# chrhansk/sleqp

Hardware: AMD Instinct MI355X
Metric: KKT factor+solve/sec (numeric refactor + 1 solve with device-controlled refinement, inputs resident in HBM) (higher is better)
Workload: dtype f64; 1 GPU; banded_n1e5_m5e4; n=100000, m=50000, N=150000, nnz_J=1000000, nnz_tril_K=1100000, nnz_L=11646539, nnz_L_stored=12226637, supernodes=569, etree_levels=10, refine_steps=1, hip_graphs=5, solves_per_factor=1, parallelism=single

## Files before the change

include/hipfact.h:

```cpp
#ifndef HIPFACT_H
#define HIPFACT_H

#include <stddef.h>
#include <stdint.h>

#ifdef __cplusplus
extern "C" {
#endif

#define HIPFACT_VERSION "0.1.0"

enum
{
  HIPFACT_OK         = 0,
  HIPFACT_EINVAL     = -1,
  HIPFACT_EDEVICE    = -2,
  HIPFACT_ESINGULAR  = -3,
  HIPFACT_ENOMEM     = -4,
  HIPFACT_ESTATE     = -5,
  HIPFACT_EINTERNAL  = -6
};

typedef struct hipfact_handle hipfact_handle;

// ... 31 lines not shown
int hipfact_solve_device_multi(hipfact_handle* h, int nrhs, const double* d_rhs, long long ld_rhs,
                               double* d_sol, long long ld_sol, double* omega);

int hipfact_solve_multi(hipfact_handle* h, int nrhs, const double* rhs, double* sol);

enum { HIPFACT_EXTRA_CONVERGED = 0, HIPFACT_EXTRA_STALLED = 1, HIPFACT_EXTRA_NONFINITE = 2, HIPFACT_EXTRA_PASS_LIMIT = 3 };
typedef struct hipfact_extra_info {
  int passes;
  int status;
  double ferr;
  double dz_rel;
  double rho;
  double omega;
} hipfact_extra_info;
int hipfact_solve_device_extra(hipfact_handle* h, const double* d_rhs, double* d_sol, hipfact_extra_info* info );
int hipfact_solve_extra(hipfact_handle* h, const double* rhs, double* sol, hipfact_extra_info* info );

int hipfact_residual_device(hipfact_handle* h, const double* d_b, const double* d_z, double* d_res, int extended);

int hipfact_solve_device_multi_extra(hipfact_handle* h, int nrhs, const double* d_rhs, long long ld_rhs, double* d_sol,
                                     long long ld_sol, hipfact_extra_info* info );
int hipfact_solve_multi_extra(hipfact_handle* h, int nrhs, const double* rhs, double* sol,
                              hipfact_extra_info* info );

int hipfact_residual_device_multi(hipfact_handle* h, int nrhs, const double* d_b, long long ld_b, const double* d_z,
                                  long long ld_z, double* d_res, long long ld_res, int extended);

enum { HIPFACT_COND_STOP_EXACT = 0,
       HIPFACT_COND_STOP_NO_GAIN = 1,
       HIPFACT_COND_STOP_PARALLEL = 2,
       HIPFACT_COND_STOP_MAX_AT_BEST = 3,
       HIPFACT_COND_STOP_REVISIT = 4,
       HIPFACT_COND_STOP_ITMAX = 5 };
typedef struct hipfact_cond_info {
  double norm1;
  double inv_norm1;
  double cond1;
  double omega;
  int exact;
  int iterations;
  int blocks;
  int column;
  int stop;
} hipfact_cond_info;
int hipfact_condition_estimate(hipfact_handle* h, int equilibrated, hipfact_cond_info* info ,
                               double* d_witness );

int hipfact_check(hipfact_handle* h);

int hipfact_synchronize(hipfact_handle* h);

int hipfact_stream(hipfact_handle* h, void** stream);


int hipfact_assemble_kkt(hipfact_handle* h, int n, int m_total, const int* j_colptr, const int* j_rowidx,
                         const double* j_vals, const int* var_index, const int* cons_index, int working_set_size,
                         int* k_nnz, int* k_colptr, int* k_rowidx, double* k_vals);


int hipfact_reduced_matrix(hipfact_handle* h, int* nnz, int* colptr, int* rowidx, double* vals);


typedef struct hipfact_spmat hipfact_spmat;

int hipfact_spmat_create(hipfact_handle* h, int num_rows, int num_cols, const int* colptr, const int* rowidx,
                         const double* vals, hipfact_spmat** out);
int hipfact_spmat_update_values(hipfact_spmat* M, const double* vals);
int hipfact_spmat_free(hipfact_spmat** M);

int hipfact_spmat_mult_vec(hipfact_spmat* M, const double* x, double* y);
int hipfact_spmat_mult_vec_trans(hipfact_spmat* M, const double* x, double* y);
int hipfact_spmat_mult_vec_sym(hipfact_spmat* M, const double* x, double* y);
int hipfact_spmat_mult_device(hipfact_spmat* M, int trans, const double* d_x, double* d_y);


int hipfact_steihaug_solve(hipfact_handle* h, hipfact_spmat* hess, const double* gradient, double trust_radius,
                           double rel_tol, int max_iter, double* newton_step, double* tr_dual, int* iterations);


typedef int (*hipfact_hess_prod_fn)(void* user, const double* direction, double* product);

enum
{
  HIPFACT_TR_STEIHAUG = 0,
  HIPFACT_TR_GLTR     = 1
};

int hipfact_tr_solve(hipfact_handle* h, int method, hipfact_spmat* hess, hipfact_hess_prod_fn prod, void* user,
                     const double* gradient, double trust_radius, double rel_tol, int max_iter, double* newton_step,
                     double* tr_dual, int* iterations);

typedef struct hipfact_tr_extra
{
  double time_limit;
  int timed_out;
  double min_rayleigh;
  double max_rayleigh;
} hipfact_tr_extra;

int hipfact_tr_solve_ex(hipfact_handle* h, int method, hipfact_spmat* hess, hipfact_hess_prod_fn prod, void* user,
                        const double* gradient, double trust_radius, double rel_tol, int max_iter, double* newton_step,
                        double* tr_dual, int* iterations, hipfact_tr_extra* extra);


typedef int (*hipfact_lsqr_prod_fn)(void* user, int trans, const double* in, double* out);

typedef struct hipfact_lsqr_op
{
  int num_residuals;
  hipfact_spmat* jac;
  hipfact_lsqr_prod_fn prod;
  void* user;
  hipfact_spmat* cons;
} hipfact_lsqr_op;

enum
{
  HIPFACT_LSQR_CONVERGED = 0,
  HIPFACT_LSQR_BOUNDARY  = 1,
  HIPFACT_LSQR_MAX_ITER  = 2,
  HIPFACT_LSQR_TIME      = 3,
  HIPFACT_LSQR_ZERO      = 4
};

typedef struct hipfact_lsqr_info
{
  double time_limit;
  int iterations;
  int status;
  int timed_out;
  double phi_bar;
} hipfact_lsqr_info;

int hipfact_lsqr_solve(hipfact_handle* h, const hipfact_lsqr_op* op, const double* rhs, double rel_tol,
                       double trust_radius, double eps, int max_iter, double* step, hipfact_lsqr_info* info);

int hipfact_tridiag_tr(int k, const double* delta, const double* gamma, double gamma0, double radius, double* h,
                       double* lambda);


int hipfact_set_option(hipfact_handle* h, const char* name, double value);

int hipfact_get_info(const hipfact_handle* h, const char* name, double* value);

int hipfact_debug_copy(hipfact_handle* h, const char* name, void* out, size_t bytes);

int hipfact_debug_pool_selftest(int callers, int rounds);

int hipfact_debug_place_rows(int m, const int* Ar_ptr, long long fill_bytes, int classes, long long* bounds, int* classes_out,
                             int* grid_out, int* blocks);
int hipfact_debug_place_items(int nfronts, const int* counts, int classes, int* order, int* lost);

int hipfact_debug_multi_slices(int u, int slice_rows, int* tile_bounds , int cap);

int hipfact_debug_extra_rule(int nblocks, int npasses, const double* dn, const double* zn, int pass_cap, int* applied,
                             int* status, double* ferr, double* rho);
int hipfact_debug_multi_extra_schedule(int ncols, int nblocks, int npasses, const double* dn, const double* zn,
                                       int pass_cap, unsigned int* open_mask, hipfact_extra_info* info);
int hipfact_debug_condest_dense(int N, const double* A, long long ld, hipfact_cond_info* info,
                                double* witness , int* history , int cap);
int hipfact_debug_condest_recorded(int N, int nrecords, const double* records, hipfact_cond_info* info);
enum {
  HIPFACT_CADENCE_FACTOR = 0,
  HIPFACT_CADENCE_SOLVE = 1,
  HIPFACT_CADENCE_VERDICT = 2,
  HIPFACT_CADENCE_JUDGE = 3,
  HIPFACT_CADENCE_RESET = 4,
  HIPFACT_CADENCE_SET_STEPS = 5,
  HIPFACT_CADENCE_SET_CHECK_EVERY = 6,
  HIPFACT_CADENCE_SET_CHECK_BACKOFF = 7,
  HIPFACT_CADENCE_SAVE = 8,
  HIPFACT_CADENCE_RESTORE = 9,
  HIPFACT_CADENCE_DEVICE_RESIDUAL = 10,
  HIPFACT_CADENCE_EVENT_WIDTH = 8,
  HIPFACT_CADENCE_ROW_WIDTH = 20
};
int hipfact_debug_refine_cadence(const int* knobs , int nevents, const double* events, long long* rows);
double hipfact_debug_dd_residual(int nterms, const double* k, const double* z, double b, int lanes);


typedef struct hipfact_plan hipfact_plan;
int hipfact_plan_create(int N, const int* colptr, const int* rowidx, const double* vals ,
                        hipfact_plan** out);
void hipfact_plan_free(hipfact_plan** plan);
const char* hipfact_plan_error(const hipfact_plan* plan);
int hipfact_plan_array(const hipfact_plan* plan, const char* name, const void** data, int64_t* len,
                       int* elem_size);
int hipfact_plan_scalar(const hipfact_plan* plan, const char* name, double* value);

#ifdef __cplusplus
}
#endif

#endif
```

sleqp_amd/_lib.py:

```python
from __future__ import annotations

import ctypes as C
import os

_HERE = os.path.dirname(os.path.abspath(__file__))
LIB_PATH = os.environ.get("HIPFACT_LIBRARY") or os.path.join(_HERE, "csrc", "libhipfact.so")

HIPFACT_OK = 0
ERRORS = {
    -1: "HIPFACT_EINVAL",
    -2: "HIPFACT_EDEVICE",
    -3: "HIPFACT_ESINGULAR",
    -4: "HIPFACT_ENOMEM",
    -5: "HIPFACT_ESTATE",
    -6: "HIPFACT_EINTERNAL",
}

SYMBOLS = [
    "hipfact_create", "hipfact_free", "hipfact_retain", "hipfact_last_error", "hipfact_last_warning", "hipfact_set_matrix", "hipfact_solve_sparse",
    "hipfact_solve_dense", "hipfact_solution", "hipfact_solution_view", "hipfact_condition", "hipfact_refactor_device",
    "hipfact_solve_device", "hipfact_solve_device_multi", "hipfact_solve_multi",
    "hipfact_condition_estimate", "hipfact_debug_condest_dense", "hipfact_debug_condest_recorded",
    "hipfact_solve_device_extra", "hipfact_solve_extra", "hipfact_residual_device", "hipfact_debug_extra_rule", "hipfact_debug_dd_residual",
    "hipfact_solve_device_multi_extra", "hipfact_solve_multi_extra", "hipfact_residual_device_multi", "hipfact_debug_multi_extra_schedule",
    "hipfact_solution_device", "hipfact_synchronize", "hipfact_check", "hipfact_stream",
    "hipfact_assemble_kkt", "hipfact_reduced_matrix", "hipfact_spmat_create", "hipfact_spmat_update_values", "hipfact_spmat_free",
    "hipfact_spmat_mult_vec", "hipfact_spmat_mult_vec_trans", "hipfact_spmat_mult_vec_sym",
    "hipfact_spmat_mult_device", "hipfact_steihaug_solve", "hipfact_tr_solve", "hipfact_tr_solve_ex", "hipfact_lsqr_solve", "hipfact_tridiag_tr", "hipfact_set_option", "hipfact_get_info", "hipfact_debug_copy", "hipfact_debug_pool_selftest",
    "hipfact_debug_place_rows", "hipfact_debug_place_items", "hipfact_debug_multi_slices", "hipfact_debug_refine_cadence", "hipfact_plan_create",
    "hipfact_plan_free", "hipfact_plan_error", "hipfact_plan_array", "hipfact_plan_scalar",
]

_lib = None


class HipfactError(RuntimeError):
    def __init__(self, code: int, message: str):
        super().__init__(f"{ERRORS.get(code, code)}: {message}")
        self.code = code


def load() -> C.CDLL:
    global _lib
    if _lib is not None:
        return _lib
    if not os.path.exists(LIB_PATH):
        raise ImportError(
            f"{LIB_PATH} not found: build the HIP extension first "
            "(python -c 'import __graft_entry__ as g; g.build()' or make -C sleqp_amd/csrc)")
    lib = C.CDLL(LIB_PATH)
    vp, ci, cd = C.c_void_p, C.c_int, C.c_double
    lib.hipfact_create.argtypes = [C.POINTER(vp), ci]
    lib.hipfact_free.argtypes = [C.POINTER(vp)]
    lib.hipfact_retain.argtypes = [vp]
    lib.hipfact_last_error.argtypes = [vp]
    lib.hipfact_last_error.restype = C.c_char_p
    lib.hipfact_last_warning.argtypes = [vp]
    lib.hipfact_last_warning.restype = C.c_char_p
    lib.hipfact_set_matrix.argtypes = [vp, ci, vp, vp, vp]
    lib.hipfact_solve_sparse.argtypes = [vp, ci, ci, vp, vp]
    lib.hipfact_solve_dense.argtypes = [vp, vp]
    lib.hipfact_solution.argtypes = [vp, vp, ci, ci]
    lib.hipfact_solution_view.argtypes = [vp, C.POINTER(vp), ci, ci]
    lib.hipfact_condition.argtypes = [vp, C.POINTER(cd)]
    lib.hipfact_refactor_device.argtypes = [vp, vp]
    lib.hipfact_solve_device.argtypes = [vp, vp, vp]
    lib.hipfact_solve_device_multi.argtypes = [vp, ci, vp, C.c_longlong, vp, C.c_longlong, vp]
    lib.hipfact_solve_multi.argtypes = [vp, ci, vp, vp]
    if hasattr(lib, "hipfact_solve_device_extra"):
        lib.hipfact_solve_device_extra.argtypes = [vp, vp, vp, vp]
        lib.hipfact_solve_extra.argtypes = [vp, vp, vp, vp]
        lib.hipfact_residual_device.argtypes = [vp, vp, vp, vp, ci]
        lib.hipfact_debug_extra_rule.argtypes = [ci, ci, vp, vp, ci, C.POINTER(ci), C.POINTER(ci), C.POINTER(cd), C.POINTER(cd)]
        lib.hipfact_debug_dd_residual.argtypes = [ci, vp, vp, cd, ci]
        lib.hipfact_debug_dd_residual.restype = cd
    if hasattr(lib, "hipfact_solve_device_multi_extra"):
        ll = C.c_longlong
        lib.hipfact_solve_device_multi_extra.argtypes = [vp, ci, vp, ll, vp, ll, vp]
        lib.hipfact_solve_multi_extra.argtypes = [vp, ci, vp, vp, vp]
        lib.hipfact_residual_device_multi.argtypes = [vp, ci, vp, ll, vp, ll, vp, ll, ci]
        lib.hipfact_debug_multi_extra_schedule.argtypes = [ci, ci, ci, vp, vp, ci, vp, vp]
    if hasattr(lib, "hipfact_condition_estimate"):
        lib.hipfact_condition_estimate.argtypes = [vp, ci, vp, vp]
        lib.hipfact_debug_condest_dense.argtypes = [ci, vp, C.c_longlong, vp, vp, vp, ci]
        lib.hipfact_debug_condest_recorded.argtypes = [ci, ci, vp, vp]
    lib.hipfact_solution_device.argtypes = [vp, C.POINTER(vp)]
    lib.hipfact_synchronize.argtypes = [vp]
    lib.hipfact_check.argtypes = [vp]
    lib.hipfact_stream.argtypes = [vp, C.POINTER(vp)]
    lib.hipfact_assemble_kkt.argtypes = [vp, ci, ci, vp, vp, vp, vp, vp, ci, C.POINTER(ci), vp, vp, vp]
    lib.hipfact_reduced_matrix.argtypes = [vp, C.POINTER(ci), vp, vp, vp]
    lib.hipfact_spmat_create.argtypes = [vp, ci, ci, vp, vp, vp, C.POINTER(vp)]
    lib.hipfact_spmat_update_values.argtypes = [vp, vp]
    lib.hipfact_spmat_free.argtypes = [C.POINTER(vp)]
    lib.hipfact_spmat_mult_vec.argtypes = [vp, vp, vp]
    lib.hipfact_spmat_mult_vec_trans.argtypes = [vp, vp, vp]
    lib.hipfact_spmat_mult_vec_sym.argtypes = [vp, vp, vp]
    lib.hipfact_spmat_mult_device.argtypes = [vp, ci, vp, vp]
    lib.hipfact_steihaug_solve.argtypes = [vp, vp, vp, cd, cd, ci, vp, C.POINTER(cd), C.POINTER(ci)]
    lib.hipfact_tr_solve.argtypes = [vp, ci, vp, vp, vp, vp, cd, cd, ci, vp, C.POINTER(cd), C.POINTER(ci)]
    lib.hipfact_tr_solve_ex.argtypes = [vp, ci, vp, vp, vp, vp, cd, cd, ci, vp, C.POINTER(cd), C.POINTER(ci), vp]
    lib.hipfact_lsqr_solve.argtypes = [vp, vp, vp, cd, cd, cd, ci, vp, vp]
    lib.hipfact_tridiag_tr.argtypes = [ci, vp, vp, cd, cd, vp, C.POINTER(cd)]
    lib.hipfact_set_option.argtypes = [vp, C.c_char_p, cd]
    lib.hipfact_debug_copy.argtypes = [vp, C.c_char_p, vp, C.c_size_t]
    lib.hipfact_debug_pool_selftest.argtypes = [ci, ci]
    lib.hipfact_get_info.argtypes = [vp, C.c_char_p, C.POINTER(cd)]
    if hasattr(lib, "hipfact_debug_place_items"):
        lib.hipfact_debug_place_rows.argtypes = [ci, vp, C.c_longlong, ci, vp, C.POINTER(ci), C.POINTER(ci), vp]
        lib.hipfact_debug_place_items.argtypes = [ci, vp, ci, vp, vp]
    if hasattr(lib, "hipfact_debug_multi_slices"):
        lib.hipfact_debug_multi_slices.argtypes = [ci, ci, vp, ci]
    if hasattr(lib, "hipfact_debug_refine_cadence"):
        lib.hipfact_debug_refine_cadence.argtypes = [vp, ci, vp, vp]
    lib.hipfact_plan_create.argtypes = [ci, vp, vp, vp, C.POINTER(vp)]
    lib.hipfact_plan_free.argtypes = [C.POINTER(vp)]
    lib.hipfact_plan_error.argtypes = [vp]
    lib.hipfact_plan_error.restype = C.c_char_p
    lib.hipfact_plan_array.argtypes = [vp, C.c_char_p, C.POINTER(vp), C.POINTER(C.c_int64), C.POINTER(ci)]
    lib.hipfact_plan_scalar.argtypes = [vp, C.c_char_p, C.POINTER(cd)]
    for name in SYMBOLS:
        if not hasattr(lib, name) and not os.environ.get("HIPFACT_LIBRARY"):
            raise ImportError(f"{LIB_PATH} lacks {name}: rebuild it (make -C sleqp_amd/csrc)")
    lib.hipfact_plan_free.restype = None
    _lib = lib
    return lib


def kernel_sources_sha16() -> str:
    import glob
    import hashlib

    d = os.path.join(os.path.dirname(os.path.abspath(__file__)), "csrc")
    h = hashlib.sha256()
    for name in sorted(glob.glob(os.path.join(d, "*.hip")) + glob.glob(os.path.join(d, "*.inc")) + glob.glob(os.path.join(d, "*.h"))):
        h.update(os.path.basename(name).encode())
        h.update(open(name, "rb").read())
    return h.hexdigest()[:16]
```

sleqp_amd/csrc/abi_options.inc:

```
enum OptionEffect {
  FX_NONE,
  FX_GRAPHS,
  FX_GRAPHS_IF_CHANGED,
  FX_PLANS,
  FX_PLANS_IF_CHANGED,
};
struct OptionRow {
  const char* name;
  const char* env;
  OptionEffect effect;
  int (*set)(hipfact_handle* h, double v);
  const char* doc;
};
#define OPT_STORE(field, conv)                 \
  [](hipfact_handle* h, double v) -> int {     \
    const auto x = (conv);                     \
    const bool changed = h->field != x;        \
    h->field = x;                              \
    return changed;                            \
  }
static const OptionRow kOptions[] = {
    {"refine_steps", "HIPFACT_REFINE", FX_GRAPHS,
     [](hipfact_handle* h, double v) -> int {
       h->refine_steps = std::max(0, (int)v);
// ... 138 lines not shown
     "0: hipfact_assemble_kkt analyses every working set on its own rows (no superset plan)"},
    {"plan_cache", nullptr, FX_NONE,
     [](hipfact_handle* h, double v) -> int {
       h->plan_cache_max = std::max(0, (int)v);
       while ((int)h->cache.size() > h->plan_cache_max) h->cache.pop_back();
       return 1;
     },
     "inactive plan states kept (LRU); 0: one pattern at a time"},
    {"profile", nullptr, FX_NONE,
     [](hipfact_handle* h, double v) -> int {
       if (h->prof.on) prof_collect(h);
       if (v < 0)
         for (int c = 0; c < PC_COUNT; ++c) h->prof.ms[c] = 0, h->prof.max_ms[c] = 0, h->prof.cnt[c] = 0;
       h->prof.tagged.clear();
       h->prof.on = v > 0;
       return 1;
     },
     "event-time every kernel class; value < 0 resets the counters"},
    {"ordering", nullptr, FX_PLANS, OPT_STORE(prm.ordering, (int)v),
     "0 nested dissection + AMD leaves (default), 1 AMD on the whole graph, 2 natural"},
    {"max_children", nullptr, FX_PLANS, OPT_STORE(prm.max_children, (int)v),
     "relaxed amalgamation keeps fronts at this many children (default 4 = what the pull extend-add takes in one block)"},
    {"force_generic", nullptr, FX_PLANS, OPT_STORE(prm.force_generic, v != 0.0),
     "1: no saddle-point structure detection, static 1 x 1 pivots on K as given (symmetric positive definite input: the PSD shim)"},
    {"dense_mode", nullptr, FX_PLANS, OPT_STORE(prm.dense_mode, std::min(2, std::max(0, (int)v))),
     "1: late elimination inside the tree (default), 2: low-rank correction, 0: off"},
    {nullptr, "HIPFACT_DATAFLOW_RETRY", FX_NONE, OPT_STORE(df_retry_every, std::max(0, (int)v)), nullptr},
    {nullptr, "HIPFACT_CHECK_LAUNCHES", FX_NONE, OPT_STORE(check_launches, v != 0.0), nullptr},
    {nullptr, "HIPFACT_SOL_SPLIT", FX_NONE, OPT_STORE(sol_split, v != 0.0), nullptr},
    {nullptr, "HIPFACT_XCD_CLASSES", FX_NONE, OPT_STORE(xcd_classes, std::max(1, std::min(XCD_CLASSES_MAX, (int)v))), nullptr},
};
#undef OPT_STORE

static void options_from_environment(hipfact_handle* h) {
  for (const OptionRow& row : kOptions)
    if (const char* s = row.env ? getenv(row.env) : nullptr) (void)row.set(h, (double)atoi(s));
}

int hipfact_set_option(hipfact_handle* h, const char* name, double value) {
  if (!h || !name) return HIPFACT_EINVAL;
  {
    bool known = false;
    const int rc = multi_set_option(h, name, value, known);
    if (known) return rc;
  }
  {
    bool known = false;
    const int rc = condest_set_option(h, name, value, known);
    if (known) return rc;
  }
  for (const OptionRow& row : kOptions) {
    if (!row.name || strcmp(name, row.name)) continue;
    const int changed = row.set(h, value);
    if (changed < 0) return changed;
    if (row.effect == FX_GRAPHS || (row.effect == FX_GRAPHS_IF_CHANGED && changed)) drop_graphs(h);
    if (row.effect == FX_PLANS || (row.effect == FX_PLANS_IF_CHANGED && changed)) invalidate_plans(h);
    return HIPFACT_OK;
  }
  h->error = std::string("unknown option: ") + name;
  return HIPFACT_EINVAL;
}

int hipfact_debug_copy(hipfact_handle* h, const char* name, void* out, size_t bytes) {
  int rc = enter(h);
  if (rc) return rc;
  if (!name || !out) return HIPFACT_EINVAL;
  auto host_copy = [&](const auto& v) {
    if (bytes > v.size() * sizeof(v[0])) {
      h->error = "hipfact_debug_copy: unknown buffer or size";
      return HIPFACT_EINVAL;
    }
    if (bytes) memcpy(out, v.data(), bytes);
    return HIPFACT_OK;
  };
  const Plan& P = h->plan;
  if (!strcmp(name, "perm")) return host_copy(P.perm);
  if (!strcmp(name, "sn_c0")) return host_copy(P.sn_c0);
  if (!strcmp(name, "sn_r")) return host_copy(P.sn_r);
  if (!strcmp(name, "sn_rowptr")) return host_copy(P.sn_rowptr);
  if (!strcmp(name, "sn_rows")) return host_copy(P.sn_rows);
  if (!strcmp(name, "sn_Loff")) return host_copy(P.sn_Loff);
  if (!strcmp(name, "late_cols")) return host_copy(P.late_cols);
  if (!strcmp(name, "sn_level")) return host_copy(P.sn_level);
  if (!strcmp(name, "dense_cols")) return host_copy(P.dense_cols);
  if (!strcmp(name, "cond_history")) return host_copy(h->cond_history);
  const DevBuf* b = nullptr;
  if (!strcmp(name, "L")) b = &h->d_L;
  else if (!strcmp(name, "U")) b = &h->d_U;
  else if (!strcmp(name, "SPf")) b = &h->d_SPf;
  else if (!strcmp(name, "sitems")) b = &h->d_sitems;
  else if (!strcmp(name, "y")) b = &h->d_y;
  else if (!strcmp(name, "xhat")) b = &h->d_xhat;
  else if (!strcmp(name, "ysol")) b = &h->d_ysol;
  else if (!strcmp(name, "uvec")) b = &h->d_uvec;
  else if (!strcmp(name, "dscale")) b = &h->d_dscale;
  else if (!strcmp(name, "Kval")) b = &h->d_Kval;
  else if (!strcmp(name, "mY")) b = &h->d_mY;
  if (!strcmp(name, "cond_d")) {
    const size_t N = (size_t)h->N_ext, off = (2 * COND_T + 3) * N * sizeof(double);
    if (!h->d_cblk.p || bytes > N * sizeof(double)) {
      h->error = "hipfact_debug_copy: unknown buffer or size";
      return HIPFACT_EINVAL;
    }
    HCHECK(h, hipStreamSynchronize(h->stream));
    HCHECK(h, hipMemcpy(out, h->d_cblk.as<char>() + off, bytes, hipMemcpyDeviceToHost));
    return HIPFACT_OK;
  }
  if (!b || !b->p || bytes > b->bytes) {
    h->error = "hipfact_debug_copy: unknown buffer or size";
    return HIPFACT_EINVAL;
  }
  HCHECK(h, hipStreamSynchronize(h->stream));
  HCHECK(h, hipMemcpy(out, b->p, bytes, hipMemcpyDeviceToHost));
  return HIPFACT_OK;
}

int hipfact_debug_place_rows(int m, const int* Ar_ptr, long long fill_bytes, int classes, long long* bounds, int* classes_out,
                             int* grid_out, int* blocks) {
  if (m < 0 || (m > 0 && !Ar_ptr) || fill_bytes < 0 || classes < 1 || classes > XCD_CLASSES_MAX || !bounds || !classes_out ||
      !grid_out || !blocks)
    return HIPFACT_EINVAL;
  ClassBounds cb;
  *grid_out = place_rows(m, Ar_ptr, (size_t)fill_bytes, classes, cb);
  *classes_out = cb.C;
  for (int g = 0; g <= cb.C; ++g) bounds[g] = cb.b[g];
  for (int g = 0; g < cb.C; ++g) class_row_blocks(cb, g, FB / RL, blocks[2 * g], blocks[2 * g + 1]);
  return HIPFACT_OK;
}
int hipfact_debug_place_items(int nfronts, const int* counts, int classes, int* order, int* lost) {
  if (nfronts < 0 || (nfronts > 0 && !counts) || classes < 1 || classes > XCD_CLASSES_MAX) return HIPFACT_EINVAL;
  long long total = 0;
  for (int f = 0; f < nfronts; ++f) {
    if (counts[f] < 0) return HIPFACT_EINVAL;
    total += counts[f];
  }
  if (total >= (1LL << 31) || (total > 0 && (!order || !lost))) return HIPFACT_EINVAL;
  std::vector<int> o, l;
  deal_items(std::vector<int>(counts, counts + nfronts), classes, o, &l);
  for (size_t i = 0; i < o.size(); ++i) {
    order[i] = o[i];
    lost[i] = l[i];
  }
  return HIPFACT_OK;
}

int hipfact_debug_multi_slices(int u, int slice_rows, int* tile_bounds, int cap) {
  if (u < 0 || !multi_slice_rows_valid(slice_rows)) return HIPFACT_EINVAL;
  const int ns = multi_nslice(u, slice_rows);
  if (tile_bounds && ns <= cap)
    for (int k = 0; k <= ns; ++k) tile_bounds[k] = multi_slice_tile(u, ns, k);
  return ns;
}

int hipfact_debug_refine_cadence(const int* knobs, int nevents, const double* events, long long* rows) {
  using namespace hipfact;
  if (!knobs || nevents < 0 || (nevents > 0 && (!events || !rows))) return HIPFACT_EINVAL;
  for (int q = 0; q < 7; ++q)
    if (knobs[q] < 0 || ((q == 1 || q >= 5) && knobs[q] > 1) || (q >= 2 && q <= 4 && knobs[q] < 1)) return HIPFACT_EINVAL;
  CadenceKnobs k{knobs[0], knobs[1] != 0, knobs[2], knobs[3], knobs[4], knobs[5] != 0, knobs[6] != 0};
  FactorCadence f;
  PlanCadence p;
  SolveCadence s;
  LiveCadence l;
  Cadence cad{f, p, s, l};
  SavedCadence saved{};
  bool have_saved = false;
  for (int e = 0; e < nevents; ++e) {
    const double* ev = events + (size_t)e * HIPFACT_CADENCE_EVENT_WIDTH;
    for (int q = 0; q < 6; ++q)
      if (!(std::fabs(ev[q]) < (double)(1 << 30)) || ev[q] != std::floor(ev[q])) return HIPFACT_EINVAL;
    const int kind = (int)ev[0], flag = (int)ev[1];
    const CtlPeek c{(int)ev[2], (int)ev[3], (int)ev[4], (int)ev[5], ev[6], ev[7]};
    const bool yes_no = flag == 0 || flag == 1;
    SolveDecision d{false, false, false, 0, 0};
    switch (kind) {
      case HIPFACT_CADENCE_FACTOR:
        if (!yes_no) return HIPFACT_EINVAL;
        cad.factor_queued(k, flag != 0, c);
        break;
      case HIPFACT_CADENCE_SOLVE:
        if (flag < 0 || flag > 3) return HIPFACT_EINVAL;
        d = cad.solve_decision(k, (flag & 1) != 0, cad.wants_peek(k) ? c : CtlPeek{-1, 0, 0, 0, 0.0, 0.0}, (flag & 2) != 0);
        if (d.flush_first) cad.verdict_flushed();
        cad.solve_queued(k, d);
        break;
      case HIPFACT_CADENCE_VERDICT:
        if (flag < 0) return HIPFACT_EINVAL;
        cad.verdict_read(k, c);
        cad.verdict_counted(c, flag);
        break;
      case HIPFACT_CADENCE_JUDGE:
        if (!yes_no) return HIPFACT_EINVAL;
        cad.judge(k, flag != 0);
        break;
      case HIPFACT_CADENCE_RESET: cad.slots_reset(); break;
      case HIPFACT_CADENCE_SET_STEPS:
        k.refine_steps = std::max(0, flag);
        cad.steps_set(k);
        break;
      case HIPFACT_CADENCE_SET_CHECK_EVERY:
        k.check_every = std::max(1, flag);
        cad.check_interval_set();
        break;
      case HIPFACT_CADENCE_SET_CHECK_BACKOFF:
        k.check_backoff = std::max(1, flag);
        cad.check_interval_set();
        break;
      case HIPFACT_CADENCE_SAVE:
        saved = cad.save();
        have_saved = true;
        break;
      case HIPFACT_CADENCE_RESTORE:
        if (!have_saved) return HIPFACT_EINVAL;
        cad.put_back(saved);
        break;
      case HIPFACT_CADENCE_DEVICE_RESIDUAL: cad.counted_device_residual(); break;
      default: return HIPFACT_EINVAL;
    }
    const long long row[HIPFACT_CADENCE_ROW_WIDTH] = {
        d.defer, d.unchecked, d.key, d.flush_first, f.refine_inline, f.inline_probe, f.wc_hint, s.check_interval_now,
        s.solves_since_check, s.num_checked, l.solve_seq, l.ctl_pending, l.decide_deferred, s.num_refined, s.num_passes,
        p.seq_at_factor, p.hint_seq_seen, p.first_factor_seq, s.last_solve_checked, cad.unchecked_solves_ok(k)};
    memcpy(rows + (size_t)e * HIPFACT_CADENCE_ROW_WIDTH, row, sizeof row);
  }
  return HIPFACT_OK;
}

int hipfact_get_info(const hipfact_handle* h, const char* name, double* value) {
  if (!h || !name || !value) return HIPFACT_EINVAL;
  const Plan& P = h->plan;
  if (!strncmp(name, "prof_", 5)) {
    prof_collect(const_cast<hipfact_handle*>(h));
    if (!strcmp(name, "prof_schur_best_flops") || !strcmp(name, "prof_schur_best_ms")) {
      double fmax = 0.0, best_rate = 0.0, bf = 0.0, bm = 0.0;
      for (auto& t : h->prof.tagged) fmax = std::max(fmax, t.first);
      for (auto& t : h->prof.tagged)
        if (t.first >= 0.5 * fmax && t.second > 0.0 && t.first / t.second > best_rate) {
          best_rate = t.first / t.second;
          bf = t.first;
          bm = t.second;
        }
      *value = !strcmp(name, "prof_schur_best_flops") ? bf : bm;
      return HIPFACT_OK;
    }
    for (int c = 0; c < PC_COUNT; ++c) {
      const size_t len = strlen(kProfNames[c]);
      if (!strncmp(name + 5, kProfNames[c], len) && name[5 + len] == '_') {
        if (!strcmp(name + 6 + len, "ms")) {
          *value = h->prof.ms[c];
          return HIPFACT_OK;
        }
        if (!strcmp(name + 6 + len, "count")) {
          *value = (double)h->prof.cnt[c];
          return HIPFACT_OK;
        }
        if (!strcmp(name + 6 + len, "max_ms")) {
          *value = h->prof.max_ms[c];
          return HIPFACT_OK;
        }
      }
    }
    return HIPFACT_EINVAL;
  }
  if (!strncmp(name, "level_", 6)) {
    const char* us = strrchr(name, '_');
    const int l = atoi(us + 1);
    if (us == name + 5 || l < 0 || l >= P.nlevels || (int)P.level_ptr.size() <= l + 1) return HIPFACT_EINVAL;
    const size_t len = (size_t)(us - (name + 6));
    double fronts = 0, ent = 0, rows = 0, flops = 0, blk = 0;
    for (int q = P.level_ptr[l]; q < P.level_ptr[l + 1]; ++q) {
      const int s = P.level_sn[q];
      const double w = P.sn_c0[s + 1] - P.sn_c0[s], r = P.sn_r[s];
      fronts += 1;
      ent += w * r - w * (w - 1) / 2;
      blk += w * (w + 1) / 2;
      rows += r;
      for (int k = 0; k < (int)w; ++k) flops += (r - k) * (r - k);
    }
    if (len == 6 && !strncmp(name + 6, "fronts", 6)) *value = fronts;
    else if (len == 3 && !strncmp(name + 6, "ent", 3)) *value = ent;
    else if (len == 3 && !strncmp(name + 6, "blk", 3)) *value = blk;
    else if (len == 4 && !strncmp(name + 6, "rows", 4)) *value = rows;
    else if (len == 5 && !strncmp(name + 6, "flops", 5)) *value = flops;
    else return HIPFACT_EINVAL;
    return HIPFACT_OK;
  }
#define INFO(key, expr)       \
  if (!strcmp(name, key)) {   \
    *value = (double)(expr);  \
    return HIPFACT_OK;        \
  }
  INFO("N", h->have_plan ? h->N_ext : P.N) INFO("n", P.n) INFO("m", P.m) INFO("saddle", P.saddle) INFO("nnzK", P.nnzK) INFO("nnzL", P.nnzL)
  INFO("nnzL_true", P.nnzL_true) INFO("flops", P.flops) INFO("flops_dense", P.flops_dense) INFO("nsuper", P.nsuper)
  INFO("nlevels", P.nlevels) INFO("nprod", P.nprod) INFO("L_bytes", P.L_size * 8.0) INFO("U_bytes", P.U_size * 8.0)
  INFO("analysis_s", P.t_total) INFO("order_s", P.t_order) INFO("symbolic_s", P.t_symbolic)
  INFO("num_perturbed", h->num_perturbed) INFO("static_pivot_runs", h->static_pivot_runs) INFO("static_pivot_shift", h->reg_delta)
  INFO("num_zero_pivots", h->info_host[INFO_ZERO_PIVOT]) INFO("num_neg_pivots", h->info_host[INFO_NEG_PIVOT])
  INFO("cache_hits", h->cache_hits) INFO("plan_swaps", h->plan_swaps) INFO("plans_cached", h->cache.size())
  INFO("no_dataflow", h->no_dataflow) INFO("dataflow_fallbacks", h->dataflow_fallbacks) INFO("turn_waits", (double)h->turn_waits) INFO("dataflow_rearmed", h->dataflow_rearmed) INFO("fused_solve", h->fused_solve) INFO("spanel_folded", h->sp_folded) INFO("solve_items", h->n_sitems) INFO("chain_levels_fused", [&] { int c = 0; for (const LevelInfo& li : h->levels) c += li.mini_cnt > 0; return c; }()) INFO("solve_panel_bytes", h->sp_bytes) INFO("spf_bytes", (double)h->d_SPf.bytes) INFO("sitem_bytes", (double)sizeof(SolveItem)) INFO("N_internal", P.N) INFO("maps_on", h->maps_on) INFO("m_struct", h->m_struct) INFO("analyses", h->analyses) INFO("num_factor", h->num_factor) INFO("cg_device_runs", h->cg_device_runs) INFO("cg_device_fallbacks", h->cg_device_fallbacks) INFO("lz_device_runs", h->lz_device_runs) INFO("lz_device_fallbacks", h->lz_device_fallbacks) INFO("lz_device_iterations", h->lz_device_iterations) INFO("lsqr_runs", h->lsqr_runs) INFO("lsqr_iters", h->lsqr_iters) INFO("dense_columns", h->nd) INFO("late_columns", P.n_late) INFO("late_rows", P.n_late_rows) INFO("m_rows", P.saddle ? P.my : P.m) INFO("vtable_rows", h->vj->rows()) INFO("vtable_retries", h->vtable_retries) INFO("dense_fallbacks", h->dense_fallbacks) INFO("dense_probes", h->dense_probes) INFO("top_block_cols", h->tb_nT) INFO("top_block_below", h->tb_nfb) INFO("top_block_levels", h->tb_levels) INFO("top_block_items", h->tb_ntf) INFO("top_block_builds", h->tb_builds) INFO("top_block_active", h->tb_valid) INFO("superset_vtable", h->superset_vtable) INFO("exact_pattern", h->exact_pattern) INFO("spmv_stream", h->spmv_stream)
  INFO("boundary_fast", h->boundary_fast) INFO("bd_count", h->bd_count) INFO("bd_stage_us", h->bd_stage_us) INFO("bd_queue_us", h->bd_queue_us) INFO("bd_rhs_us", h->bd_rhs_us) INFO("bd_device_us", h->bd_device_us) INFO("bd_d2h_us", h->bd_d2h_us) INFO("bd_wait_us", h->bd_wait_us) INFO("bd_copyout_us", h->bd_copyout_us)
  INFO("multi_solves", h->multi_solves) INFO("multi_cols", h->multi_cols) INFO("multi_blocks", h->multi_blocks)
  INFO("multi_passes", h->multi_passes) INFO("multi_single_cols", h->multi_single_cols) INFO("multi_failed_col", h->multi_failed_col)
  INFO("multi_sliced_fronts", h->mitems_for < 0 ? 0 : h->n_mcut) INFO("multi_slice_items", h->mitems_for < 0 ? 0 : h->n_mslices) INFO("multi_slice_rows", h->multi_slice_rows)
  INFO("cond_estimates", h->cond_estimates) INFO("cond_blocks", h->cond_blocks) INFO("cond_last", h->cond_last) INFO("condition_estimate", h->condition_estimate)
  INFO("extra_solves", h->extra_solves) INFO("extra_passes", h->extra_passes) INFO("extra_last_status", h->extra_last_status)
  INFO("extra_multi_solves", h->extra_multi_solves) INFO("extra_multi_cols", h->extra_multi_cols) INFO("extra_multi_passes", h->extra_multi_passes)
  INFO("num_solve", h->num_solve) INFO("num_refined", h->solve_cad.num_refined) INFO("refine_adaptive", h->refine_adaptive)
  INFO("num_passes", h->solve_cad.num_passes) INFO("last_omega", h->last_ctl.omega) INFO("last_iters", h->last_ctl.iters)
  INFO("last_status", h->last_ctl.status) INFO("last_tol", h->last_ctl.tol) INFO("kappa_est", h->last_ctl.kappa)
  INFO("refine_inline", h->factor_cad.refine_inline) INFO("refine_tol", h->refine_tol) INFO("equilibrate", h->equilibrate)
  INFO("factor_top_level", h->ftop_level) INFO("factor_top_count", h->ftop_count) INFO("solve_timeouts", h->h_info.p ? h->h_info.as<int>()[INFO_TIMEOUT] : 0)
  INFO("top_level", 1 << 30)
  INFO("use_graph", h->use_graph) INFO("num_graphs", h->graphs.size()) INFO("max_r", P.max_r) INFO("max_w", P.max_w) INFO("refine_steps", h->refine_steps)
  INFO("schur_flops_max_level", h->schur_flops_max)
  INFO("chain_pairs", h->n_pairs)
  INFO("xupd_fused", h->xupd_fused ? 1 : 0)
  INFO("rhs_in_tree", h->last_rhs_in_tree) INFO("xupd_in_tree", h->last_xupd_in_tree) INFO("xupd_blocks_launched", h->last_xupd_blocks)
  INFO("solve_sliced_fronts", h->n_sliced) INFO("solve_resorted_levels", h->n_resorted) INFO("tree_solve", tree_solve(h))
  INFO("refine_check_every", h->refine_check_every) INFO("refine_check_interval", h->solve_cad.check_interval_now) INFO("num_checked", h->solve_cad.num_checked)
  INFO("device", h->device) INFO("nnzM", P.Mi.size()) INFO("nnzA", P.Ar_src.size())
  INFO("rows_total", P.sn_rows.size()) INFO("ent_fused", h->ent_fused) INFO("ent_split", h->ent_split)
  INFO("rows_fused", h->rows_fused) INFO("rows_split", h->rows_split)
  INFO("long_row_segments", h->n_rseg) INFO("row_scale_blocks", row_scale_in_sequence(h) ? h->rs_grid : 0)
  INFO("arena_fill_bytes", arena_fill_bytes(P))
  INFO("xcd_classes", h->xcd_classes) INFO("dealt_multi_item_fronts", h->dealt_multi) INFO("long_prod_segments", h->n_lprod)
  INFO("active_bounds", h->maps_on ? h->n_bounds : 0)
  INFO("values_in_place",
       h->have_plan && (!h->from_jacobian || (virtual_current(h) && h->vj->identity))) INFO("inactive_rows", h->maps_on ? h->n_inactive : 0)
#undef INFO
  return HIPFACT_EINVAL;
}
```

sleqp_amd/csrc/device_types.h:

```cpp
#pragma once
#include <cstdint>

namespace hipfact {

struct SnDesc {
  long long Loff;
  long long Uoff;
  long long uoff;
  long long rowoff;
  long long reloff;
  int c0;
  int w;
  int r;
  int parent;
  int child_begin;
  int child_end;
  int pad0;
  int pad1;
};

constexpr int MAXCH = 4;
struct PullDesc {
  long long Uoff[MAXCH];
  long long reloff[MAXCH];
  int invoff[MAXCH];
  int uc[MAXCH];
  int n;
  int next;
  int pad[2];
};

struct FrontItem {
  long long Loff, Uoff;
  int w, r;
  int part;
  int nchild;
  PullDesc pd;
};

struct PairDesc {
  long long Loff_a, Uoff_g;
  int w_a, r_a, rowoff_a;
  int u_g, off_g;
};

struct TopFItem {
  FrontItem it;
  int role;
  int front;
  int part2;
  int nwait;
  int wait_id[MAXCH];
  int wait_cnt[MAXCH];
  int target;
  int crows;
  int prows;
  int sidx, scount;
  int post;
  long long xoff;
  int head;
  int wait_head[MAXCH];
};

struct SolveItem {
  long long spf, spd;
  long long uoff, rowoff;
  int c0, w, r, nchild;
  int Qf, Ef, Pb, Eb;
  long long c_uoff[MAXCH];
  int c_invoff[MAXCH];
  long long Loff;
  int xbegin, xend;
  int a0, a1, sl, nsl;
  long long poff;
  int plevel, pad_;
};
constexpr int LONG_ROW = 1024;
constexpr int LONG_COL = 256;
constexpr int LONG_SEG = 2048;
struct LongSeg {
  int id;
  int begin, end;
  int idx, nseg;
  int uid;
  int poff;
  int pad;
};
struct LongProd {
  long long e;
  long long begin, end;
  int idx, nseg, uid, poff;
};
constexpr int XCD_CLASSES_MAX = 16;
struct ClassBounds {
  long long b[XCD_CLASSES_MAX + 1];
  int C, pad;
};
#ifdef __HIP__
#define HIPFACT_HD __host__ __device__
#else
#define HIPFACT_HD
#endif
HIPFACT_HD inline void class_row_blocks(const ClassBounds& cb, int g, int rpb, int& rb0, int& nrb) {
  rb0 = (int)((cb.b[g] + rpb - 1) / rpb);
  nrb = (int)((cb.b[g + 1] + rpb - 1) / rpb) - rb0;
}
struct TopBlockItem {
  long long off;
  int r0, nr;
  int Q, E;
};
struct TopFront {
  int item;
  int parent;
  int tl0;
  int pad;
};
struct TopChunk {
  int front;
  int j0;
};
constexpr int TOP_CB = 4;
constexpr int TOP_LDS = 7 * 1024 + 512;
constexpr int SPMV_NNZ = 2048;
constexpr int SPMV_T = 256;
constexpr int TREE_LDS = 2 * 1024 + 8;
struct TopBlockIn {
  int nT, ntf;
  const TopBlockItem* __restrict__ items;
  const double* __restrict__ XTf;
  const int* __restrict__ tpos;
  const int* __restrict__ gptr;
  const long long* __restrict__ gsrc;
  double* __restrict__ xhatT2;
  double* __restrict__ tT2;
  int ntr;
  unsigned int* __restrict__ gathered2;
  int ltop;
};
constexpr int SOLVE_PREFETCH = 32;

enum { INFO_ZERO_PIVOT = 0, INFO_NEG_PIVOT = 1, INFO_TIMEOUT = 2, INFO_TIMEOUT_WG = 3, INFO_WORDS = 4 };
constexpr int INFO_BYTES = INFO_WORDS * 4 + 32;

}
```

sleqp_amd/csrc/hipfact.hip:

```cpp
#include <hip/hip_runtime.h>

#include <dlfcn.h>

#include <algorithm>
#include <atomic>
#include <chrono>
#include <cmath>
#include <cstdio>
#include <cstdlib>
#include <cstring>
#include <memory>
#include <new>
#include <string>
#include <condition_variable>
#include <functional>
#include <mutex>
#include <thread>
#include <unordered_map>
#include <vector>

#include "../../include/hipfact.h"
#include "device_types.h"
#include "plan.h"
#include "tridiag_tr.h"

#include "kernel_types.h"
#include "kernels_decl.h"
#include "xcd_place.h"
#include "multi_slices.h"
#include "refine_cadence.h"
#include "condest_rule.h"
#include "dd_arith.h"

#include "runtime_types.inc"
#include "runtime_plan.inc"
#include "runtime_queue.inc"
#include "runtime_multi.inc"
#include "runtime_extra.inc"
#include "runtime_multi_extra.inc"
#include "runtime_condest.inc"

extern "C" {
#include "abi_core.inc"
#include "abi_multi.inc"
#include "abi_extra.inc"
#include "abi_multi_extra.inc"
#include "abi_condest.inc"
#include "abi_working_set.inc"
#include "abi_krylov.inc"
#include "abi_options.inc"
}
```

sleqp_amd/csrc/kernels_factor_top.inc:

```

__device__ __forceinline__ void flag_wait_ge(int* __restrict__ addr, int target, int* __restrict__ info) {
  if (threadIdx.x == 0) {
    int spins = 0;
    while (__hip_atomic_load(addr, __ATOMIC_RELAXED, __HIP_MEMORY_SCOPE_AGENT) < target) {
      __builtin_amdgcn_s_sleep(2);
      if (++spins > (1 << 22)) {
        atomicAdd(&info[INFO_TIMEOUT], 1);
        break;
      }
    }
    __builtin_amdgcn_fence(__ATOMIC_ACQUIRE, "agent");
    asm volatile("s_waitcnt vmcnt(0)" ::: "memory");
  }
  __syncthreads();
}

__device__ __forceinline__ void flag_publish_add(int* __restrict__ addr) {
  asm volatile("s_waitcnt vmcnt(0)" ::: "memory");
  __syncthreads();
  if (threadIdx.x == 0) {
    FACTOR_RELEASE_FENCE();
    asm volatile("s_waitcnt vmcnt(0)" ::: "memory");
    __hip_atomic_fetch_add(addr, 1, __ATOMIC_RELAXED, __HIP_MEMORY_SCOPE_AGENT);
  }
}

__device__ __forceinline__ void dev_build_solve_panel(const SolveItem& T, const double* __restrict__ L,
                                                      double* __restrict__ SPf, double* lds);

__global__ __launch_bounds__(512) void k_factor_top(const TopFItem* __restrict__ items, double* __restrict__ L,
                                                   double* __restrict__ U, int* __restrict__ info,
                                                   const int* __restrict__ inv, const int* __restrict__ rel,
                                                   int* __restrict__ bdone, int* __restrict__ cdone,
                                                   int* __restrict__ ddone, double* __restrict__ xarena,
                                                   const SolveItem* __restrict__ sitems, double* __restrict__ SPf) {
  extern __shared__ __attribute__((aligned(16))) double lds[];
  const TopFItem& T = items[blockIdx.x];
  const FrontItem& S = T.it;
  TRW(0);
#ifdef HIPFACT_TRACE
  if (threadIdx.x == 0 && blockIdx.x < TRACE_WGS) g_trace[blockIdx.x * 8 + 7] = T.role * 100000 + T.front;
#endif
  if (T.role == 3) {
    if (T.nwait) {
      if (threadIdx.x == 0) {
        int spins = 0;
        while ((__hip_atomic_load(&bdone[T.front], __ATOMIC_RELAXED, __HIP_MEMORY_SCOPE_AGENT) & 15) < 1 ||
               __hip_atomic_load(&cdone[T.front], __ATOMIC_RELAXED, __HIP_MEMORY_SCOPE_AGENT) < T.target) {
          __builtin_amdgcn_s_sleep(8);
          if (++spins > (1 << 22)) {
            atomicAdd(&info[INFO_TIMEOUT], 1);
            break;
          }
        }
        __builtin_amdgcn_fence(__ATOMIC_ACQUIRE, "agent");
        asm volatile("s_waitcnt vmcnt(0)" ::: "memory");
      }
      __syncthreads();
    }
    TRW(1);
    dev_build_solve_panel(sitems[S.part], L, SPf, lds);
#ifdef HIPFACT_TRACE
    __syncthreads();
#endif
    TRW(2);
    return;
  }
  FrontCtx c = make_ctx(S, L, U, lds);
  c.wt = true;
  c.Xa = T.post ? xarena + T.xoff : nullptr;
  const PullCtx pc = make_pull(S.pd, U, inv, rel, 1);
  ChildWait cw;
  cw.n = T.nwait;
  cw.info = info;
#pragma unroll
  for (int ch = 0; ch < MAXCH; ++ch) {
    cw.addr[ch] = ddone + T.wait_id[ch];
    cw.target[ch] = T.wait_cnt[ch];
  }
  if (T.role == 0) {
    int* hdone = ddone + (ddone - cdone);
#pragma unroll
    for (int ch = 0; ch < MAXCH; ++ch)
      if (T.wait_head[ch] > 0 && ch < T.nwait && T.wait_cnt[ch] > 0) {
        cw.addr[ch] = hdone + T.wait_id[ch];
        cw.target[ch] = T.wait_head[ch];
      }
  }
  if (T.role == 0) {
    dev_pivot_block<false, false, true>(c, info, 15, pc, cw);
    dev_store_pivot_block(c);
    TRW(2);
    flag_publish_add(&bdone[T.front]);
    TRW(3);
    if (T.sidx > 0) {
      const SolveItem& Q = sitems[T.sidx - 1];
      const int w = c.w, r = c.r, lda = c.lda;
      const int lane = threadIdx.x & 63, wave = threadIdx.x >> 6;
      double* __restrict__ sf = SPf + Q.spf;
      double* __restrict__ sd = SPf + Q.spd;
      for (int k = wave; k < w; k += 8)
        for (int i = k + lane; i < w; i += 64) sf[(long long)k * r + i] = (i == k) ? 1.0 : c.A[i + k * lda];
      for (int i = threadIdx.x; i < w; i += blockDim.x) sd[i] = 1.0 / c.dd[i];
    }
  } else if (T.role == 1) {
    TRW(5);
    cw.wait();
    int* invl = reinterpret_cast<int*>(c.A + c.wp * c.lda);
#pragma unroll
    for (int ch = 0; ch < MAXCH; ++ch)
      if (ch < pc.n)
        for (int k = threadIdx.x; k < c.wp; k += blockDim.x) invl[ch * c.wp + k] = (k < c.w) ? pc.inv[ch][k] : -1;
    const int wv = threadIdx.x >> 6;
    const int cstep = T.prows == 64 ? 2 : 1;
    const int R0 = c.w + T.prows * S.part + 16 * (cstep == 2 ? (wv >> 1) : wv);
    double pv[8][4];
    int cis[MAXCH];
    if (c.Xa) {
      const bool mine = 16 * wv < T.prows;
      const int R1 = c.w + T.prows * S.part + 16 * wv;
      const int Rs = mine ? R1 : c.r;
      dev_panel_rows_load<true>(c, Rs, pc, pv, cis);
      __syncthreads();
      dev_panel_rows_gather<true>(c, pc, invl, pv, cis);
      TRW(1);
      dev_panel_rows_subst_posted(c, Rs, pv, mine && R1 < c.r, S.part == 0, info);
      TRW(2);
      flag_publish_add(&cdone[T.front]);
      TRW(3);
      return;
    }
    dev_panel_rows_load(c, R0, pc, pv, cis);
    __syncthreads();
    dev_panel_rows_gather(c, pc, invl, pv, cis);
    if (c.Xa) {
      dev_panel_rows_product_posted(c, R0, pv, cstep, cstep == 2 ? (wv & 1) : 0, R0 < c.r, info);
    } else {
      flag_wait_ge(&bdone[T.front], 1, info);
      TRW(1);
      dev_load_pivot_block(c, true, true);
      if (R0 < c.r) dev_panel_rows_product<true, true>(c, R0, pv, cstep, cstep == 2 ? (wv & 1) : 0);
    }
    TRW(2);
    flag_publish_add(&cdone[T.front]);
    TRW(3);
  } else if (T.role == 4) {
#define FUSED_ARGS c, S.part >> 16, S.part & 0xffff, pc, cw, info, &bdone[T.front], &cdone[T.front], &ddone[T.front], T.target
    if (T.crows == 32) {
      if (c.nbk == 6)
        dev_fused_tile<32, 6>(FUSED_ARGS);
      else
        dev_fused_tile<32, 0>(FUSED_ARGS);
    } else {
      if (c.nbk == 6)
        dev_fused_tile<64, 6>(FUSED_ARGS);
      else
        dev_fused_tile<64, 0>(FUSED_ARGS);
    }
#undef FUSED_ARGS
  } else {
    cw.wait();
    if (T.crows == 64) {
      dev_schur_tile32(c, S.part >> 16, S.part & 0xffff, pc, &cdone[T.front], T.target, info);
    } else {
      const int team = threadIdx.x >> 8;
      const int ij = team ? T.part2 : S.part;
      double* SI = c.A + (size_t)team * (2 * 64 * KC + 64 * MAXCH);
      dev_schur_tile<false>(c, SI, SI + 64 * KC, ij < 0 ? -1 : (ij >> 16), ij & 0xffff, S.nchild == 0, pc,
                            threadIdx.x & 255, &cdone[T.front], T.target, info);
    }
    if (c.Xa)
      for (int e = T.sidx * 512 + threadIdx.x; e < c.wp * c.wp; e += T.scount * 512) sent_f64(c.Xa + e);
    TRW(2);
    flag_publish_add(&ddone[T.front]);
    if (T.head && threadIdx.x == 0)
      __hip_atomic_fetch_add(ddone + (ddone - cdone) + T.front, 1, __ATOMIC_RELAXED, __HIP_MEMORY_SCOPE_AGENT);
    TRW(3);
  }
}
```

sleqp_amd/csrc/kernels_front_pivot.inc:

```

struct FrontCtx {
  int w, r, u, wp, nbk, lda;
  double* P;
  double* Us;
  double* dd;
  double* A;
  double* Yp;
  double* Xa;
  bool wt;
};

__device__ __forceinline__ double panel_entry(const FrontCtx& c, long long off) { return c.P[off]; }

template <class Desc>
__device__ __forceinline__ FrontCtx make_ctx(const Desc& S, double* L, double* U, double* lds) {
  FrontCtx c;
  c.w = S.w;
  c.r = S.r;
  c.u = S.r - S.w;
  c.wp = (S.w + 15) & ~15;
  c.nbk = c.wp >> 4;
  c.lda = c.wp + 1;
  c.P = L + S.Loff;
  c.Us = U + S.Uoff;
// ... 213 lines not shown
      }
    }
}
__device__ __forceinline__ void pivot_offsets_stage1(const PullCtx& pc, const int* invb, int wp, int i1, int kq1,
                                                     int (&o1)[MAXCH][4]) {
#pragma unroll
  for (int ch = 0; ch < MAXCH; ++ch) {
    const int* ib = invb + ch * wp;
    const int uc = pc.uc[ch];
    const int ci = (ch < pc.n && i1 < wp) ? ib[i1] : -1;
#pragma unroll
    for (int q = 0; q < 4; ++q) {
      const int ck = (ch < pc.n) ? ib[kq1 + 4 * q] : -1;
      o1[ch][q] = (ci >= 0 && ck >= 0 && ci >= ck) ? ci + ck * uc : -1;
    }
  }
}
__device__ __forceinline__ bool stage2_elem(int wp, int wave, int lane, int s, int j, int& i, int& k) {
  const int npairs = (wp - 16) >> 1;
  const int p = (wave - 1) + 7 * j;
  const int t = lane + 64 * s;
  const int ka = 16 + p, kb = wp - 1 - p;
  const int len1 = wp - ka;
  const bool first = t < len1;
  k = first ? ka : kb;
  i = first ? ka + t : kb + (t - len1);
  return wave >= 1 && p < npairs && t < wp - 15;
}
__device__ __forceinline__ void pivot_gather_stage2_from(const PullCtx& pc, const int* invb, int wp, int lane, int wave,
                                                         double (&v)[2][8], int cfirst) {
#pragma unroll
  for (int c0 = 0; c0 < MAXCH; c0 += 2)
    if (c0 >= cfirst && c0 < pc.n) {
      double g[2][2][8];
#pragma unroll
      for (int cc = 0; cc < 2; ++cc) {
        const int ch = c0 + cc;
        const bool has = ch < pc.n;
        const double* __restrict__ Uc = has ? pc.Uc[ch] : pc.Uc[c0];
        const int uc = has ? pc.uc[ch] : 0;
        const int* ib = invb + (has ? ch : c0) * wp;
#pragma unroll
        for (int s2 = 0; s2 < 2; ++s2)
#pragma unroll
          for (int j = 0; j < 8; ++j) {
            int i, k;
            const bool valid = stage2_elem(wp, wave, lane, s2, j, i, k);
            const int ci = (valid && has) ? ib[i] : -1;
            const int ck = (valid && has) ? ib[k] : -1;
            const bool ok = ci >= 0 && ck >= 0;
            const double gv = Uc[ok ? ci + (long long)ck * uc : 0];
            g[cc][s2][j] = ok ? gv : 0.0;
          }
      }
#pragma unroll
      for (int cc = 0; cc < 2; ++cc)
#pragma unroll
        for (int s2 = 0; s2 < 2; ++s2)
#pragma unroll
          for (int j = 0; j < 8; ++j) v[s2][j] += g[cc][s2][j];
    }
}
__device__ __forceinline__ void pivot_gather_stage2(const PullCtx& pc, const int* invb, int wp, int lane, int wave,
                                                    double (&v)[2][8]) {
  pivot_gather_stage2_from(pc, invb, wp, lane, wave, v, 0);
}
__device__ __forceinline__ void pivot_offsets_stage2(const PullCtx& pc, const int* invb, int wp, int lane, int wave,
                                                     int (&o2)[2][2][8]) {
#pragma unroll
  for (int cc = 0; cc < 2; ++cc) {
    const bool has = cc < pc.n;
    const int uc = pc.uc[cc];
    const int* ib = invb + cc * wp;
#pragma unroll
    for (int s2 = 0; s2 < 2; ++s2)
#pragma unroll
      for (int j = 0; j < 8; ++j) {
        int i, k;
        const bool valid = stage2_elem(wp, wave, lane, s2, j, i, k);
        const int ci = (valid && has) ? ib[i] : -1;
        const int ck = (valid && has) ? ib[k] : -1;
        o2[cc][s2][j] = (ci >= 0 && ck >= 0) ? ci + ck * uc : -1;
      }
  }
}

__device__ __forceinline__ void flag_wait_ge(int* __restrict__ addr, int target, int* __restrict__ info);
struct ChildWait {
  int n;
  int* addr[MAXCH];
  int target[MAXCH];
  int* info;
  __device__ __forceinline__ void wait() const {
    bool any = false;
#pragma unroll
    for (int ch = 0; ch < MAXCH; ++ch) any = any || (ch < n && target[ch] > 0);
    if (!any) return;
    if (threadIdx.x == 0) {
#pragma unroll
      for (int ch = 0; ch < MAXCH; ++ch)
        if (ch < n && target[ch] > 0) {
          int spins = 0;
          while (__hip_atomic_load(addr[ch], __ATOMIC_RELAXED, __HIP_MEMORY_SCOPE_AGENT) < target[ch]) {
            __builtin_amdgcn_s_sleep(2);
            if (++spins > (1 << 22)) {
              atomicAdd(&info[INFO_TIMEOUT], 1);
              break;
            }
          }
        }
      __builtin_amdgcn_fence(__ATOMIC_ACQUIRE, "agent");
      asm volatile("s_waitcnt vmcnt(0)" ::: "memory");
    }
    __syncthreads();
  }
};
__device__ __forceinline__ ChildWait no_wait() {
  ChildWait cw;
  cw.n = 0;
  cw.info = nullptr;
#pragma unroll
  for (int ch = 0; ch < MAXCH; ++ch) {
    cw.addr[ch] = nullptr;
    cw.target[ch] = 0;
  }
  return cw;
}

__device__ __forceinline__ void lds_flag_set(int* f, int v) {
  asm volatile("s_waitcnt lgkmcnt(0)" ::: "memory");
  __hip_atomic_store(f, v, __ATOMIC_RELAXED, __HIP_MEMORY_SCOPE_WORKGROUP);
}
__device__ __forceinline__ void lds_flag_add(int* f) {
  asm volatile("s_waitcnt lgkmcnt(0)" ::: "memory");
  if ((threadIdx.x & 63) == 0) __hip_atomic_fetch_add(f, 1, __ATOMIC_RELAXED, __HIP_MEMORY_SCOPE_WORKGROUP);
}
__device__ __forceinline__ void lds_flag_wait_ge(int* f, int v, int* __restrict__ info) {
  int spins = 0;
  while (__hip_atomic_load(f, __ATOMIC_RELAXED, __HIP_MEMORY_SCOPE_WORKGROUP) < v) {
    __builtin_amdgcn_s_sleep(1);
    if (++spins > (1 << 22)) {
      if ((threadIdx.x & 63) == 0) atomicAdd(&info[INFO_TIMEOUT], 1);
      break;
    }
  }
  asm volatile("s_waitcnt lgkmcnt(0)" ::: "memory");
}
enum { PF_DIAG = 0, PF_STAGE2 = 1, PF_LRDY = 2, PF_UPD = 10, PF_WORDS = 18 };

__device__ __forceinline__ void dev_pivot_chain(const FrontCtx& c, double* dinv, int* flags, int* __restrict__ info);

template <bool ROWINV, bool CHAIN = false, bool V2 = false>
__device__ __forceinline__ void dev_pivot_block(const FrontCtx& c, int* __restrict__ info, int phases, const PullCtx& pc,
                                                const ChildWait& cw, const PullMore pm = no_more()) {
  const int tid = threadIdx.x, lane = tid & 63, wave = tid >> 6;
  const int nw = blockDim.x >> 6;
  const int li = lane & 15, lk = lane >> 4;
  const int w = c.w, r = c.r, wp = c.wp, nbk = c.nbk, lda = c.lda;
  double* A = c.A;
  double* dd = c.dd;
  double* Yp = c.Yp;
  double* scratch = V2 ? Yp : Yp + 16 * lda;
  int* pflags = reinterpret_cast<int*>(Yp + wp);
  if (V2 && tid < PF_WORDS) pflags[tid] = 0;
  const double* __restrict__ P = c.P;
  if (pc.n > 0) {
    int* invb = reinterpret_cast<int*>(Yp + 16 * lda + 32);
    int iv[MAXCH];
#pragma unroll
    for (int ch = 0; ch < MAXCH; ++ch) iv[ch] = (ch < pc.n && tid < w) ? pc.inv[ch][tid] : -1;
    const int i1 = tid & 127, kq1 = tid >> 7;
    double v1[4];
#pragma unroll
    for (int q = 0; q < 4; ++q) {
      const int k = kq1 + 4 * q;
      v1[q] = (i1 == k) ? 1.0 : 0.0;
      if (i1 < w && k < w) v1[q] = (i1 >= k) ? panel_entry(c, i1 + (long long)k * r) : 0.0;
    }
    double v[2][8];
#pragma unroll
    for (int s2 = 0; s2 < 2; ++s2)
#pragma unroll
      for (int j = 0; j < 8; ++j) {
        int i, k;
        const bool valid = stage2_elem(wp, wave, lane, s2, j, i, k);
        v[s2][j] = (valid && i == k) ? 1.0 : 0.0;
        if (valid && i < w && k < w) v[s2][j] = panel_entry(c, i + (long long)k * r);
      }
#pragma unroll
    for (int ch = 0; ch < MAXCH; ++ch)
      if (ch < pc.n && tid < wp) invb[ch * wp + tid] = iv[ch];
    __syncthreads();
    if constexpr (!CHAIN) {
      int o1[MAXCH][4], o2[2][2][8];
      pivot_offsets_stage1(pc, invb, wp, i1, kq1, o1);
      if (wave >= 1) pivot_offsets_stage2(pc, invb, wp, lane, wave, o2);
      TRW(5);
      cw.wait();
      TRW(1);
      double g1[MAXCH][4], g2[2][2][8];
#pragma unroll
      for (int ch = 0; ch < MAXCH; ++ch)
        if (ch < pc.n) {
#pragma unroll
          for (int q = 0; q < 4; ++q) g1[ch][q] = pc.Uc[ch][o1[ch][q] >= 0 ? o1[ch][q] : 0];
        }
      if (wave >= 1) {
#pragma unroll
        for (int cc = 0; cc < 2; ++cc)
          if (cc < pc.n) {
#pragma unroll
            for (int s2 = 0; s2 < 2; ++s2)
#pragma unroll
              for (int j = 0; j < 8; ++j) g2[cc][s2][j] = pc.Uc[cc][o2[cc][s2][j] >= 0 ? o2[cc][s2][j] : 0];
          }
      }
#pragma unroll
      for (int ch = 0; ch < MAXCH; ++ch)
        if (ch < pc.n) {
#pragma unroll
          for (int q = 0; q < 4; ++q) v1[q] += o1[ch][q] >= 0 ? g1[ch][q] : 0.0;
        }
      if (i1 < wp) {
#pragma unroll
        for (int q = 0; q < 4; ++q) A[i1 + (kq1 + 4 * q) * lda] = v1[q];
      }
      __syncthreads();
      TRP(0);
      if (wave == 0) {
        if (!(phases & 32)) dev_diag_block(c, scratch, 0, info);
        TRP(1);
      } else {
#pragma unroll
        for (int cc = 0; cc < 2; ++cc)
          if (cc < pc.n) {
#pragma unroll
            for (int s2 = 0; s2 < 2; ++s2)
#pragma unroll
              for (int j = 0; j < 8; ++j) v[s2][j] += o2[cc][s2][j] >= 0 ? g2[cc][s2][j] : 0.0;
          }
        if (pc.n > 2) pivot_gather_stage2_from(pc, invb, wp, lane, wave, v, 2);
#pragma unroll
        for (int s2 = 0; s2 < 2; ++s2)
#pragma unroll
          for (int j = 0; j < 8; ++j) {
            int i, k;
            if (stage2_elem(wp, wave, lane, s2, j, i, k)) A[i + k * lda] = v[s2][j];
          }
      }
      if (!V2) __syncthreads();
    } else {
      cw.wait();
      pivot_gather_stage1(pc, invb, wp, i1, kq1, v1);
      if (wave >= 1) pivot_gather_stage2(pc, invb, wp, lane, wave, v);
      for (int nx = pc.next; nx >= 0;) {
        const PullCtx px = make_pull(pm.more[nx], pm.U, pm.inv, pm.rel, 1);
        __syncthreads();
#pragma unroll
        for (int ch = 0; ch < MAXCH; ++ch)
          if (tid < wp) invb[ch * wp + tid] = (ch < px.n && tid < w) ? px.inv[ch][tid] : -1;
        __syncthreads();
        pivot_gather_stage1(px, invb, wp, i1, kq1, v1);
        if (wave >= 1) pivot_gather_stage2(px, invb, wp, lane, wave, v);
        nx = px.next;
      }
      if (i1 < wp) {
#pragma unroll
        for (int q = 0; q < 4; ++q) A[i1 + (kq1 + 4 * q) * lda] = v1[q];
      }
      if (wave >= 1) {
#pragma unroll
        for (int s2 = 0; s2 < 2; ++s2)
#pragma unroll
          for (int j = 0; j < 8; ++j) {
            int i, k;
            if (stage2_elem(wp, wave, lane, s2, j, i, k)) A[i + k * lda] = v[s2][j];
          }
      }
      __syncthreads();
      if (wave == 0 && !(phases & 32)) dev_diag_block(c, scratch, 0, info);
      __syncthreads();
    }
  } else {
    for (int kk = wave; kk < wp; kk += 8 * nw)
      for (int i = lane; i < wp; i += 64) {
        double v[8];
#pragma unroll
        for (int q = 0; q < 8; ++q) {
          const int k = kk + nw * q;
          v[q] = (i == k) ? 1.0 : 0.0;
          if (i < w && k < w) v[q] = (i >= k) ? panel_entry(c, i + (long long)k * r) : 0.0;
        }
#pragma unroll
        for (int q = 0; q < 8; ++q) {
          const int k = kk + nw * q;
          if (k < wp) A[i + k * lda] = v[q];
        }
      }
    __syncthreads();
    if (wave == 0 && !(phases & 32)) dev_diag_block(c, scratch, 0, info);
    __syncthreads();
  }

  d4_t xpend = {0.0, 0.0, 0.0, 0.0};
  int xrow = -1, xcol = -1;
  if constexpr (V2) {
    if (wave >= 1) lds_flag_add(&pflags[PF_STAGE2]);
    dev_pivot_chain(c, scratch, pflags, info);
    TRW(4);
    __syncthreads();
  }
  for (int kb = 0; kb < (V2 ? 0 : nbk); ++kb) {
    const int k0 = kb << 4;
    if (ROWINV && xrow >= 0) {
#pragma unroll
      for (int q = 0; q < 4; ++q) {
        const int row = 16 * xrow + lk + 4 * q, col = 16 * xcol + li;
        A[row + col * lda] = -xpend[q];
        if (row < w) {
          gst(c.wt, &c.P[row + (long long)col * r], -xpend[q]);
          if (c.Xa) post_f64(c.Xa + row + col * c.wp, -xpend[q]);
        }
      }
      xrow = -1;
    }
    if (!(phases & 64))
      for (int I = kb + 1 + wave; I < nbk; I += nw) {
        d4_t acc = {0.0, 0.0, 0.0, 0.0};
#pragma unroll
        for (int s = 0; s < 4; ++s) {
          const double av = A[(16 * I + li) + (k0 + 4 * s + lk) * lda];
          const double bv = A[(k0 + li) + (k0 + 4 * s + lk) * lda];
          acc = MFMA_F64(av, bv, acc);
        }
        const double dinv = scratch[li];
#pragma unroll
        for (int q = 0; q < 4; ++q) {
          const int row = 16 * I + lk + 4 * q;
          Yp[row + li * lda] = acc[q];
          A[row + (k0 + li) * lda] = acc[q] * dinv;
        }
      }
    __syncthreads();
    if (kb + 1 < nbk) {
// ... 573 lines not shown
```

sleqp_amd/csrc/kernels_front_update.inc:

```
template <bool X_IN_LDS, bool RECIP = false>
__device__ __forceinline__ void dev_panel_solve(const FrontCtx& c, int blk, int blk_stride, const PullCtx& pc,
                                                const int* invl) {
  const int wave = threadIdx.x >> 6;
  const int RB = 16 * (blockDim.x >> 6);
  for (int R0 = c.w + RB * blk + 16 * wave; R0 < c.r; R0 += RB * blk_stride) {
    double pv[8][4];
    int cis[MAXCH];
    dev_panel_rows_load(c, R0, pc, pv, cis);
    dev_panel_rows_finish<X_IN_LDS, RECIP>(c, R0, pc, invl, pv, cis);
  }
}

constexpr int KC = 32;
constexpr int SCB = 64;
__device__ __forceinline__ void schur_tile_gather(const PullCtx& pc, const int* invs, int i0, int j0, int li, int lk,
                                                  double (&uv)[2][2][4]) {
#pragma unroll
  for (int ch = 0; ch < MAXCH; ++ch)
    if (ch < pc.n) {
      const double* __restrict__ Uc = pc.Uc[ch];
      const int uc = pc.uc[ch];
      const int* iv = invs + 128 * ch;
      int ci[2], cj[2][4];
#pragma unroll
      for (int y = 0; y < 2; ++y) ci[y] = iv[i0 + 16 * y + li];
#pragma unroll
      for (int x = 0; x < 2; ++x)
#pragma unroll
        for (int q = 0; q < 4; ++q) cj[x][q] = iv[64 + j0 + 16 * x + lk + 4 * q];
      double g[2][2][4];
#pragma unroll
      for (int x = 0; x < 2; ++x)
#pragma unroll
        for (int y = 0; y < 2; ++y)
#pragma unroll
          for (int q = 0; q < 4; ++q) {
            const bool ok = ci[y] >= 0 && cj[x][q] >= 0 && ci[y] >= cj[x][q];
            const double gv = Uc[ok ? ci[y] + (long long)cj[x][q] * uc : 0];
            g[x][y][q] = ok ? gv : 0.0;
          }
#pragma unroll
      for (int x = 0; x < 2; ++x)
#pragma unroll
        for (int y = 0; y < 2; ++y)
#pragma unroll
          for (int q = 0; q < 4; ++q) uv[x][y][q] += g[x][y][q];
    }
}

template <bool DD_IN_LDS, bool CHAIN = false>
__device__ __forceinline__ void dev_schur_tile(const FrontCtx& c, double* SI, double* SJ, int I, int J, bool assign,
                                               const PullCtx& pc, const int tid, int* wait_addr = nullptr,
                                               int wait_target = 0, int* info = nullptr,
                                               const PullMore pm = no_more()) {
  const int lane = tid & 63, wave = tid >> 6;
  const int li = lane & 15, lk = lane >> 4;
  const int w = c.w, r = c.r, u = c.u;
  const double* __restrict__ P21 = c.P + w;
  const int wi = wave & 1, wj = wave >> 1;
  const bool ghost = I < 0;
  const bool idle = ghost || (I == J && wi < wj);
  const int i0 = 32 * wi, j0 = 32 * wj;
  d4_t acc[2][2];
#pragma unroll
  for (int x = 0; x < 2; ++x)
#pragma unroll
    for (int y = 0; y < 2; ++y) acc[x][y] = (d4_t){0.0, 0.0, 0.0, 0.0};
  double uv[2][2][4];
#pragma unroll
  for (int x = 0; x < 2; ++x)
#pragma unroll
    for (int y = 0; y < 2; ++y) {
      const int i = 64 * I + i0 + 16 * y + li;
#pragma unroll
      for (int q = 0; q < 4; ++q) {
        const int j = 64 * J + j0 + 16 * x + lk + 4 * q;
        uv[x][y][q] = (!assign && !idle && pc.n == 0 && i < u && j < u && i >= j) ? c.Us[i + (long long)j * u] : 0.0;
      }
    }
  int* invs = reinterpret_cast<int*>(SJ + 64 * KC);
  int ivr[2] = {-1, -1};
  if (pc.n > 0) {
#pragma unroll
    for (int h = 0; h < 2; ++h) {
      const int ch = (tid >> 7) + 2 * h, idx = tid & 127;
      const int gi = (idx < 64) ? 64 * I + idx : 64 * J + idx - 64;
#pragma unroll
      for (int cc = 0; cc < MAXCH; ++cc)
        if (cc == ch && cc < pc.n && gi < u && !ghost) ivr[h] = pc.inv[cc][w + gi];
    }
  }
  if (wait_addr) {
    if (pc.n > 0) {
      invs[tid] = ivr[0];
      invs[tid + 256] = ivr[1];
    }
    __syncthreads();
    if (!idle) schur_tile_gather(pc, invs, i0, j0, li, lk, uv);
    TRW(5);
    flag_wait_ge(wait_addr, wait_target, info);
    TRW(1);
  }
  const int si = tid & 63;
  const bool iok = !ghost && (64 * I + si) < u, jok = !ghost && (64 * J + si) < u;
  const double* __restrict__ pi = P21 + 64 * I + si;
  const double* __restrict__ pj = P21 + 64 * J + si;
  for (int kc0 = 0; kc0 < w; kc0 += KC) {
    const int kcn = min(KC, w - kc0);
    __syncthreads();
    for (int kk = tid >> 6; kk < kcn; kk += 32) {
      double vi[8], vj[8], vd[8];
#pragma unroll
      for (int q = 0; q < 8; ++q) {
        const int k = kk + 4 * q;
        vi[q] = (iok && k < kcn) ? pi[(long long)(kc0 + k) * r] : 0.0;
        vj[q] = (jok && k < kcn) ? pj[(long long)(kc0 + k) * r] : 0.0;
        vd[q] = (k < kcn) ? (DD_IN_LDS ? c.dd[kc0 + k] : c.P[(kc0 + k) + (long long)(kc0 + k) * r]) : 0.0;
      }
#pragma unroll
      for (int q = 0; q < 8; ++q) {
        const int k = kk + 4 * q;
        if (k < kcn) {
          SI[k * 64 + si] = vi[q];
          SJ[k * 64 + si] = vj[q] * vd[q];
        }
      }
    }
    if (kc0 == 0 && pc.n > 0 && !wait_addr) {
      invs[tid] = ivr[0];
      invs[tid + 256] = ivr[1];
    }
    __syncthreads();
    if (!idle) {
      const int k4 = kcn & ~3;
      for (int k0 = 0; k0 < k4; k0 += 4) {
        const int kk = (k0 + lk) * 64;
        const double a0 = SJ[kk + j0 + li], a1 = SJ[kk + j0 + 16 + li];
        const double b0 = SI[kk + i0 + li], b1 = SI[kk + i0 + 16 + li];
        acc[0][0] = MFMA_F64(a0, b0, acc[0][0]);
        acc[0][1] = MFMA_F64(a0, b1, acc[0][1]);
        acc[1][0] = MFMA_F64(a1, b0, acc[1][0]);
        acc[1][1] = MFMA_F64(a1, b1, acc[1][1]);
      }
      if (k4 < kcn) {
        const bool kok = (k4 + lk) < kcn;
        const int kk = (k4 + lk) * 64;
        const double a0 = kok ? SJ[kk + j0 + li] : 0.0, a1 = kok ? SJ[kk + j0 + 16 + li] : 0.0;
        const double b0 = kok ? SI[kk + i0 + li] : 0.0, b1 = kok ? SI[kk + i0 + 16 + li] : 0.0;
        acc[0][0] = MFMA_F64(a0, b0, acc[0][0]);
        acc[0][1] = MFMA_F64(a0, b1, acc[0][1]);
        acc[1][0] = MFMA_F64(a1, b0, acc[1][0]);
        acc[1][1] = MFMA_F64(a1, b1, acc[1][1]);
      }
    }
  }
  if (!wait_addr) {
    if (!idle) schur_tile_gather(pc, invs, i0, j0, li, lk, uv);
    for (int nx = CHAIN ? pc.next : -1; nx >= 0;) {
      const PullCtx px = make_pull(pm.more[nx], pm.U, pm.inv, pm.rel, 1);
      __syncthreads();
#pragma unroll
      for (int h = 0; h < 2; ++h) {
        const int ch = (tid >> 7) + 2 * h, idx = tid & 127;
        const int gi = (idx < 64) ? 64 * I + idx : 64 * J + idx - 64;
        int val = -1;
#pragma unroll
        for (int cc = 0; cc < MAXCH; ++cc)
          if (cc == ch && cc < px.n && gi < u && !ghost) val = px.inv[cc][w + gi];
        invs[tid + 256 * h] = val;
      }
      __syncthreads();
      if (!idle) schur_tile_gather(px, invs, i0, j0, li, lk, uv);
      nx = px.next;
    }
  }
  if (idle) return;
#pragma unroll
  for (int x = 0; x < 2; ++x)
#pragma unroll
    for (int y = 0; y < 2; ++y) {
      const int i = 64 * I + i0 + 16 * y + li;
#pragma unroll
      for (int q = 0; q < 4; ++q) {
        const int j = 64 * J + j0 + 16 * x + lk + 4 * q;
        if (i < u && j < u && i >= j) {
          gst(c.wt, &c.Us[i + (long long)j * u], uv[x][y][q] - acc[x][y][q]);
        }
      }
    }
}

__device__ __forceinline__ void dev_schur_tile32(const FrontCtx& c, int I, int J, const PullCtx& pc,
                                                 int* __restrict__ wait_addr, int wait_target,
                                                 int* __restrict__ info) {
  const int tid = threadIdx.x, lane = tid & 63, wave = tid >> 6;
  const int li = lane & 15, lk = lane >> 4;
  const int w = c.w, r = c.r, u = c.u;
  const double* __restrict__ P21 = c.P + w;
  double* SI = c.A;
  double* SJ = c.A + 32 * c.wp;
  const int wi = wave & 1, wj = (wave >> 1) & 1;
  const bool mm = wave < 4 && !(I == J && wi < wj);
  double uv[4] = {0.0, 0.0, 0.0, 0.0};
  const int gi = 32 * I + 16 * wi + li;
  if (mm) {
#pragma unroll
    for (int ch = 0; ch < MAXCH; ++ch)
      if (ch < pc.n) {
        const int ci = (gi < u) ? pc.inv[ch][w + gi] : -1;
        int cj[4];
#pragma unroll
        for (int q = 0; q < 4; ++q) {
          const int gj = 32 * J + 16 * wj + lk + 4 * q;
          cj[q] = (gj < u) ? pc.inv[ch][w + gj] : -1;
        }
        double g[4];
#pragma unroll
        for (int q = 0; q < 4; ++q) {
          const bool ok = ci >= 0 && cj[q] >= 0 && ci >= cj[q];
          const double gv = pc.Uc[ch][ok ? ci + (long long)cj[q] * pc.uc[ch] : 0];
          g[q] = ok ? gv : 0.0;
        }
#pragma unroll
        for (int q = 0; q < 4; ++q) uv[q] += g[q];
      }
  }
  TRW(5);
  flag_wait_ge(wait_addr, wait_target, info);
  TRW(1);
  {
    double v[16], d[16];
#pragma unroll
    for (int t = 0; t < 16; ++t) {
      const int e = tid + 512 * t;
      const int k = e >> 6, row = e & 31;
      const bool js = (e >> 5) & 1;
      const int g = js ? 32 * J + row : 32 * I + row;
      v[t] = (k < w && g < u) ? P21[g + (long long)k * r] : 0.0;
      d[t] = (k < w && js) ? c.P[k + (long long)k * r] : 1.0;
    }
#pragma unroll
    for (int t = 0; t < 16; ++t) {
      const int e = tid + 512 * t;
      const int k = e >> 6, row = e & 31;
      if (k < c.wp) {
        if ((e >> 5) & 1)
          SJ[k * 32 + row] = v[t] * d[t];
        else
          SI[k * 32 + row] = v[t];
      }
    }
  }
  __syncthreads();
  if (!mm) return;
  d4_t acc = {0.0, 0.0, 0.0, 0.0};
  for (int k0 = 0; k0 < w; k0 += 4) {
    const int kk = (k0 + lk) * 32;
    acc = MFMA_F64(SJ[kk + 16 * wj + li], SI[kk + 16 * wi + li], acc);
  }
  if (gi < u) {
#pragma unroll
    for (int q = 0; q < 4; ++q) {
      const int gj = 32 * J + 16 * wj + lk + 4 * q;
      if (gj < u && gi >= gj) gst(c.wt, &c.Us[gi + (long long)gj * u], uv[q] - acc[q]);
    }
  }
}

__global__ __launch_bounds__(FB) void k_factor_level(const SnDesc* __restrict__ sn,
                                                     const int* __restrict__ level_sn, double* __restrict__ L,
                                                     double* __restrict__ U, const int* __restrict__ rel,
                                                     const int* __restrict__ child_idx, int* __restrict__ info,
                                                     int phases) {
  extern __shared__ __attribute__((aligned(16))) double lds[];
  const SnDesc S = sn[level_sn[blockIdx.x]];
  const FrontCtx c = make_ctx(S, L, U, lds);
  if (!(phases & 2)) return;
  PullCtx nopull;
  nopull.n = 0;
  dev_pivot_block<false>(c, info, phases, nopull, no_wait());
  dev_store_pivot_block(c);
  if (!(phases & 4)) return;
  {
    for (int k = threadIdx.x; k < c.wp; k += blockDim.x) c.Yp[k] = 1.0 / c.dd[k];
    __syncthreads();
    FrontCtx cr = c;
    cr.dd = c.Yp;
    dev_panel_solve<true, true>(cr, 0, 1, nopull, nullptr);
  }
  __syncthreads();
  if (c.u > 0 && (phases & 8)) {
    double* SI = c.A;
    double* SJ = c.A + 64 * KC;
    const int nt = (c.u + 63) >> 6;
    for (int I = 0; I < nt; ++I)
      for (int J = 0; J <= I; ++J) dev_schur_tile<true>(c, SI, SJ, I, J, S.child_begin == S.child_end, nopull, threadIdx.x);
  }
}

__global__ __launch_bounds__(1024) void k_front_assemble(const SnDesc* __restrict__ sn, const int* __restrict__ items,
                                                       int nparts, double* __restrict__ L, double* __restrict__ U,
                                                       const int* __restrict__ rel,
                                                       const int* __restrict__ child_idx) {
  extern __shared__ __attribute__((aligned(16))) double lds[];
  const SnDesc S = sn[items[2 * blockIdx.x]];
  FrontCtx c = make_ctx(S, L, U, nullptr);
  dev_assemble(S, c, sn, U, rel, child_idx, items[2 * blockIdx.x + 1], nparts, reinterpret_cast<int*>(lds));
}

// ... 237 lines not shown
```

sleqp_amd/csrc/runtime_plan.inc:

```

static void prof_begin(hipfact_handle* h, int cls) {
  Prof& p = h->prof;
  if (!p.on) return;
  if (p.used + 2 > p.ev.size()) {
    hipEvent_t a, b;
    if (hipEventCreate(&a) != hipSuccess || hipEventCreate(&b) != hipSuccess) return;
    p.ev.push_back(a);
    p.ev.push_back(b);
  }
  p.cls.resize(p.ev.size() / 2);
  p.fl.resize(p.ev.size() / 2);
  p.cls[p.used / 2] = cls;
  p.fl[p.used / 2] = p.next_fl;
  p.next_fl = 0.0;
  (void)hipEventRecord(p.ev[p.used], h->stream);
}
static void prof_end(hipfact_handle* h) {
  Prof& p = h->prof;
  if (!p.on || p.used + 2 > p.ev.size()) return;
  (void)hipEventRecord(p.ev[p.used + 1], h->stream);
  p.used += 2;
}
static void prof_collect(hipfact_handle* h) {
  Prof& p = h->prof;
// ... 288 lines not shown
      auto item = [&](int s, int part) {
        FrontItem it;
        memset(&it, 0, sizeof(it));
        it.Loff = sn[s].Loff;
        it.Uoff = sn[s].Uoff;
        it.w = sn[s].w;
        it.r = sn[s].r;
        it.part = part;
        it.nchild = sn[s].child_end - sn[s].child_begin;
        it.pd = pulls[s];
        return it;
      };
      std::vector<int> order(P.level_sn.begin() + P.level_ptr[l], P.level_sn.begin() + P.level_ptr[l + 1]);
      std::stable_sort(order.begin(), order.end(), [&](int a, int b) {
        const long long wa = sn[a].w, wb = sn[b].w;
        return wa != wb ? wa > wb : sn[a].r > sn[b].r;
      });
      li.itB = (long long)fitems.size();
      for (int s : order) fitems.push_back(item(s, 0));
      li.itC = (long long)fitems.size();
      {
        long long blocks128 = 0;
        for (int q = P.level_ptr[l]; q < P.level_ptr[l + 1]; ++q) {
          const int s = P.level_sn[q];
          blocks128 += (P.sn_r[s] - (P.sn_c0[s + 1] - P.sn_c0[s]) + 127) / 128;
        }
        li.panel_threads = (blocks128 < h->panel_small_below) ? 256 : 512;
      }
      std::vector<FrontItem> plain;
      std::vector<int> per_front, dealt;
      auto emit_by_class = [&]() {
        if (deal_items(per_front, h->xcd_classes, dealt))
          for (int c : per_front) h->dealt_multi += c > 1;
        for (int i : dealt) fitems.push_back(plain[(size_t)i]);
        plain.clear();
        per_front.clear();
      };
      const int prow = li.panel_threads / 4;
      for (int s : order) {
        const int u = P.sn_r[s] - (P.sn_c0[s + 1] - P.sn_c0[s]);
        per_front.push_back((u + prow - 1) / prow);
        for (int b = 0; b < (u + prow - 1) / prow; ++b) {
          plain.push_back(item(s, b));
          ++li.nC;
        }
      }
      emit_by_class();
      li.itD = (long long)fitems.size();
      li.compactD = false;
      li.pair = 0;
      if (order.size() == 1) {
        const int s = order[0];
        const long long u = P.sn_r[s] - (P.sn_c0[s + 1] - P.sn_c0[s]), nt = (u + 63) / 64;
        if (pair_role[s] == 1) {
          const int par = P.sn_parent[s];
          const long long ntc = std::min(nt, (long long)((sn[par].w + 63) / 64));
          li.compactD = true;
          li.pair = 1;
          fitems.push_back(item(s, (int)(-(ntc + 1))));
          li.nD = (int)(ntc * (ntc + 1) / 2 + (nt - ntc) * ntc);
          const double cc = 64.0 * (double)ntc;
          li.pair_flops_done = 2.0 * sn[s].w * ((double)u * cc - 0.5 * cc * cc);
          li.schur_flops_full = li.schur_flops;
          li.schur_flops = li.pair_flops_done;
        } else if (pair_role[s] == 2) {
          const int a = P.child_idx[P.child_ptr[s]], g = pair_g[s];
          li.compactD = true;
          li.pair = 2;
          fitems.push_back(item(s, -1));
          li.nD = (int)(nt * (nt + 1) / 2);
          li.pd.Loff_a = sn[a].Loff;
          li.pd.w_a = sn[a].w;
          li.pd.r_a = sn[a].r;
          li.pd.rowoff_a = sn[s].w;
          li.pd.Uoff_g = sn[g].Uoff;
          li.pd.u_g = sn[g].r - sn[g].w;
          li.pd.off_g = sn[a].w + sn[s].w;
          const LevelInfo& la = h->levels[P.sn_level[a]];
          li.schur_flops += la.schur_flops_full - la.pair_flops_done;
        } else if (nt * (nt + 1) / 2 >= 1024 && nt * (nt + 1) / 2 < (1LL << 31)) {
          li.compactD = true;
          fitems.push_back(item(s, -1));
          li.nD = (int)(nt * (nt + 1) / 2);
        }
      }
      for (int s : order) {
        if (li.compactD) break;
        const int u = P.sn_r[s] - (P.sn_c0[s + 1] - P.sn_c0[s]);
        const int nt = (u + 63) / 64;
        per_front.push_back(nt * (nt + 1) / 2);
        for (int I = 0; I < nt; ++I)
          for (int J = 0; J <= I; ++J) {
            plain.push_back(item(s, (I << 16) | J));
            ++li.nD;
          }
      }
      emit_by_class();
    }
  }
  h->ent_fused = h->ent_split = h->rows_fused = h->rows_split = 0;
  for (int l = 0; l < P.nlevels; ++l)
    for (int q = P.level_ptr[l]; q < P.level_ptr[l + 1]; ++q) {
      const int s = P.level_sn[q];
      const double w = P.sn_c0[s + 1] - P.sn_c0[s], r = P.sn_r[s];
      const double ent = w * r - w * (w - 1) / 2;
      (h->levels[l].split ? h->ent_split : h->ent_fused) += ent;
      (h->levels[l].split ? h->rows_split : h->rows_fused) += r;
    }
  if ((rc = upload(h, h->d_items, items))) return rc;
  if ((rc = upload(h, h->d_fitems, fitems))) return rc;
  auto slice_rows = [&](int w2) {
    const int fwd = 1024 / ((w2 + SOLVE_PREFETCH - 1) / SOLVE_PREFETCH);
    const int bwd = SOLVE_PREFETCH * std::max(1, 1024 / w2);
    return std::max(w2 + 16, std::min({fwd, bwd, 1024}));
  };
  std::vector<int> it_front, it_sl, it_nsl, it_a0, it_a1, first_item(ns, 0);
  std::vector<int> solve_order(P.level_sn.begin(), P.level_sn.begin() + ns);
  if (h->solve_sorted)
    for (int l = 0; l < P.nlevels; ++l)
      std::stable_sort(solve_order.begin() + P.level_ptr[l], solve_order.begin() + P.level_ptr[l + 1], [&](int a, int b) {
        return (long long)sn[a].r * sn[a].w > (long long)sn[b].r * sn[b].w;
      });
  h->n_resorted = 0;
  for (int l = 0; l < P.nlevels; ++l)
    h->n_resorted += !std::equal(solve_order.begin() + P.level_ptr[l], solve_order.begin() + P.level_ptr[l + 1],
                                 P.level_sn.begin() + P.level_ptr[l]);
  for (int q = 0; q < ns; ++q) {
    const int s2 = solve_order[q];
    const int w2 = std::max(1, sn[s2].w), u2 = sn[s2].r - sn[s2].w;
    const int cap = slice_rows(w2);
    first_item[s2] = (int)it_front.size();
    std::vector<std::pair<int, int>> cuts;
    const int q1 = std::max(1, 1024 / std::max(1, sn[s2].r));
    const bool whole = sn[s2].r <= 1024 && (w2 + q1 - 1) / q1 <= h->solve_whole_max;
    if (sn[s2].r <= cap || whole || !h->solve_slices) {
      cuts.push_back({0, u2});
    } else {
      const int first = std::max(16, (cap - w2) & ~15), rest = std::max(16, std::min(cap, 1024 - w2) & ~15);
      cuts.push_back({0, std::min(u2, first)});
      for (int a = cuts.back().second; a < u2; a += rest) cuts.push_back({a, std::min(u2, a + rest)});
    }
    for (size_t sl = 0; sl < cuts.size(); ++sl) {
      it_front.push_back(s2);
      it_sl.push_back((int)sl);
      it_nsl.push_back((int)cuts.size());
      it_a0.push_back(cuts[sl].first);
      it_a1.push_back(cuts[sl].second);
    }
  }
  const int nit = (int)it_front.size();
  {
    h->ftop_level = 1 << 30;
    h->ftop_count = 0;
    int lvl = P.nlevels;
    while (lvl > 0) {
      const LevelInfo& li = h->levels[lvl - 1];
      int mch = 0;
      for (int q = P.level_ptr[lvl - 1]; q < P.level_ptr[lvl]; ++q)
        mch = std::max(mch, P.child_ptr[P.level_sn[q] + 1] - P.child_ptr[P.level_sn[q]]);
      int mu = 0;
      for (int q = P.level_ptr[lvl - 1]; q < P.level_ptr[lvl]; ++q)
        mu = std::max(mu, P.sn_r[P.level_sn[q]] - (P.sn_c0[P.level_sn[q] + 1] - P.sn_c0[P.level_sn[q]]));
      if (!(li.count <= h->factor_top_max && h->pull_max_children > 0 && mch <= MAXCH &&
            P.nlevels - lvl < h->factor_top_levels && mu <= h->factor_top_max_u))
        break;
      --lvl;
    }
    h->sp_folded = false;
    h->mini_x_bytes = 0;
    if (P.nlevels - lvl >= 2 && h->factor_top_max > 0) {
      size_t sp_lds_pre = 0;
      bool fold = h->solve_fused && h->spanel_fold && ns > 0;
      {
        int wmax = 1;
        for (int s2 = 0; s2 < ns; ++s2) {
          fold = fold && sn[s2].w >= 1 && (h->solve_slices || sn[s2].r <= 1024);
          wmax = std::max(wmax, sn[s2].w);
        }
        sp_lds_pre = solve_panel_lds(wmax);
        fold = fold && sp_lds_pre <= 160 * 1024;
      }
      auto ntiles = [&](int s) {
        const long long u = sn[s].r - sn[s].w, nt = (u + 63) / 64;
        return nt * (nt + 1) / 2;
      };
      auto ntiles32 = [&](int s) {
        const long long u = sn[s].r - sn[s].w, nt = (u + 31) / 32;
        return nt * (nt + 1) / 2;
      };
      auto panel_rows = [&](int count) {
        return (count <= h->factor_top_post || count <= h->factor_top_fine) ? 64 : 128;
      };
      std::vector<TopFItem> tf;
      std::vector<size_t> level_end, panel_end;
      size_t lds = 0;
      std::vector<long long> xoff(ns, 0);
      long long xsize = 0;
      for (int l = lvl; l < P.nlevels; ++l)
        for (int q = P.level_ptr[l]; q < P.level_ptr[l + 1]; ++q) {
          const int s = P.level_sn[q];
          const long long wp = (sn[s].w + 15) & ~15;
          xoff[s] = xsize;
          xsize += wp * wp;
        }
      h->mini_x_off = xsize;
      for (int l = 0; l < lvl; ++l) {
        LevelInfo& lm = h->levels[l];
        lm.mini_cnt = 0;
        if (!(h->chain_fuse && lm.split && lm.pull && !lm.chain && lm.count == 1)) continue;
        const int s = P.level_sn[P.level_ptr[l]];
        if (sn[s].r - sn[s].w < 512 || sn[s].child_end - sn[s].child_begin > MAXCH) continue;
        const long long wp = (sn[s].w + 15) & ~15;
        xoff[s] = xsize;
        xsize += wp * wp;
        lm.mini_cnt = -1;
      }
      h->mini_x_bytes = (size_t)(xsize - h->mini_x_off) * sizeof(double);
      HCHECK(h, h->d_xarena.ensure(std::max<size_t>((size_t)xsize * sizeof(double), 16)));
      HCHECK(h, hipMemsetAsync(h->d_xarena.p, 0xFF, std::max<size_t>((size_t)xsize * sizeof(double), 16), h->stream));
      std::vector<char> lfused(P.nlevels, 0);
      auto fused_rows = [&](int l) { return h->levels[l].count <= h->factor_top_fused32 ? 32 : 64; };
      auto nfused = [&](int s) {
        const long long sr = fused_rows(P.sn_level[s]), u = sn[s].r - sn[s].w, nt = (u + sr - 1) / sr;
        return nt * (nt + 1) / 2;
      };
      auto head_rows = [&](int ch) {
        const int par = sn[ch].parent;
        if (par < 0) return 0;
        const int uc = sn[ch].r - sn[ch].w;
        const int* rl = P.rel.data() + P.rel_ptr[ch];
        return (int)(std::lower_bound(rl, rl + uc, sn[par].w) - rl);
      };
      auto is_head_tile = [&](int s, int I, int tile) { return I * tile < head_rows(s); };
      for (int l = lvl; l < P.nlevels; ++l) {
        const LevelInfo& li = h->levels[l];
        bool ok = li.count <= h->factor_top_post && li.count <= h->factor_top_fused;
        for (int q = P.level_ptr[l]; q < P.level_ptr[l + 1] && ok; ++q)
          ok = sn[P.level_sn[q]].r - sn[P.level_sn[q]].w <= h->factor_top_fused_u && sn[P.level_sn[q]].w <= 112;
        lfused[l] = ok ? 1 : 0;
      }
      for (int l = lvl; l < P.nlevels; ++l) {
        const LevelInfo& li = h->levels[l];
        lds = std::max({lds, li.lds_pivot, li.lds_panel});
        const bool fine = li.count <= h->factor_top_fine;
        auto base = [&](int s, int role, int part) {
          TopFItem t;
          memset(&t, 0, sizeof(t));
          t.it.Loff = sn[s].Loff;
          t.it.Uoff = sn[s].Uoff;
          t.it.w = sn[s].w;
          t.it.r = sn[s].r;
          t.it.part = part;
          t.it.nchild = sn[s].child_end - sn[s].child_begin;
          t.it.pd = pulls[s];
          t.role = role;
          t.front = s;
          t.part2 = part;
          t.nwait = t.it.nchild;
          for (int k = 0; k < t.nwait; ++k) {
            const int ch = P.child_idx[sn[s].child_begin + k];
            t.wait_id[k] = ch;
            t.wait_cnt[k] = P.sn_level[ch] >= lvl ? (int)(lfused[P.sn_level[ch]] ? nfused(ch)
                                                         : h->levels[P.sn_level[ch]].count <= h->factor_top_fine ? ntiles32(ch)
                                                                                                               : (ntiles(ch) + 1) / 2)
                                                  : 0;
            t.wait_head[k] = 0;
            const int cl = P.sn_level[ch];
            if (role == 0 && h->factor_top_head && cl >= lvl && !lfused[cl]) {
              const bool cfine = h->levels[cl].count <= h->factor_top_fine;
              const int tile = cfine ? 32 : 64, uc = sn[ch].r - sn[ch].w, nt = (uc + tile - 1) / tile;
              int cnt = 0, idx = 0;
              bool cur = false;
              for (int I = 0; I < nt; ++I)
                for (int J = 0; J <= I; ++J, ++idx) {
                  cur = cur || is_head_tile(ch, I, tile);
                  if (cfine || (idx & 1) || idx == nt * (nt + 1) / 2 - 1) {
                    cnt += cur;
                    cur = false;
                  }
                }
              t.wait_head[k] = cnt;
            }
          }
          t.crows = fine ? 64 : 128;
          t.post = li.count <= h->factor_top_post;
          t.prows = panel_rows(li.count);
          t.xoff = xoff[s];
          t.target = (sn[s].r - sn[s].w + t.prows - 1) / t.prows;
          return t;
        };
        std::vector<int> wide_first(P.level_sn.begin() + P.level_ptr[l], P.level_sn.begin() + P.level_ptr[l + 1]);
        std::stable_sort(wide_first.begin(), wide_first.end(), [&](int a, int b) {
          return sn[a].w != sn[b].w ? sn[a].w > sn[b].w : sn[a].r > sn[b].r;
        });
        std::vector<int> narrow_first(wide_first.rbegin(), wide_first.rend());
        for (int s : wide_first) {
          tf.push_back(base(s, 0, 0));
          const size_t wp = (size_t)((sn[s].w + 15) & ~15);
          lds = std::max(lds, (wp + 2 * (size_t)(2 * 64 * 32 + 64 * MAXCH)) * sizeof(double));
        }
        if (lfused[l]) {
          static const int fused_order = getenv("HIPFACT_FUSED_ORDER") ? atoi(getenv("HIPFACT_FUSED_ORDER")) : 0;
          for (int s : (fused_order ? wide_first : narrow_first)) {
            const int sr = fused_rows(l), nt = (sn[s].r - sn[s].w + sr - 1) / sr;
            const size_t wp = (size_t)((sn[s].w + 15) & ~15);
            for (int I = 0; I < nt; ++I)
              for (int J = 0; J <= I; ++J) {
                TopFItem t = base(s, 4, (I << 16) | J);
                t.crows = sr;
                t.target = (int)nfused(s);
                tf.push_back(t);
              }
            lds = std::max(lds, (wp + wp * (wp + 1) + 4096) * sizeof(double) + (size_t)MAXCH * wp * sizeof(int));
          }
          panel_end.push_back(tf.size());
          level_end.push_back(tf.size());
          continue;
        }
        for (int s : narrow_first) {
          const int u = sn[s].r - sn[s].w;
          const int crows = panel_rows(li.count);
          for (int b = 0; b < (u + crows - 1) / crows; ++b) tf.push_back(base(s, 1, b));
        }
        panel_end.push_back(tf.size());
        for (int pass = 0; pass < 2; ++pass)
          for (int s : narrow_first) {
            const int u = sn[s].r - sn[s].w, nt = fine ? (u + 31) / 32 : (u + 63) / 64;
            std::vector<int> tiles;
            for (int I = 0; I < nt; ++I)
              for (int J = 0; J <= I; ++J) tiles.push_back((I << 16) | J);
            const int stride = fine ? 1 : 2;
            for (size_t k = 0; k < tiles.size(); k += stride) {
              const int t2 = tiles[std::min(k + 1, tiles.size() - 1)];
              const bool hd = h->factor_top_head && (is_head_tile(s, tiles[k] >> 16, fine ? 32 : 64) ||
                                                     (!fine && is_head_tile(s, t2 >> 16, 64)));
              if (hd != (pass == 0)) continue;
              TopFItem t = base(s, 2, tiles[k]);
              t.part2 = fine ? -1 : t2;
              t.sidx = (int)(k / stride);
              t.scount = (int)((tiles.size() + stride - 1) / stride);
              t.head = hd ? 1 : 0;
              tf.push_back(t);
            }
          }
        level_end.push_back(tf.size());
      }
      if (fold) {
        std::vector<TopFItem> out;
        out.reserve(tf.size() + nit);
        int qnext = 0;
        auto filler = [&](int q) {
          const int s = it_front[q];
          TopFItem t;
          memset(&t, 0, sizeof(t));
          t.it.Loff = sn[s].Loff;
          t.it.w = sn[s].w;
          t.it.r = sn[s].r;
          t.it.part = q;
          t.role = 3;
          t.front = s;
          t.part2 = -1;
          if (P.sn_level[s] >= lvl) {
            const int crows = panel_rows(h->levels[P.sn_level[s]].count);
            t.nwait = 1;
            t.target = lfused[P.sn_level[s]] ? (int)nfused(s) : (sn[s].r - sn[s].w + crows - 1) / crows;
          }
          return t;
        };
        std::vector<char> own(ns, 0);
        for (TopFItem& t : tf)
          if (t.role == 0 && t.it.r == t.it.w) {
            t.sidx = first_item[t.front] + 1;
            own[t.front] = 1;
          }
        auto skip_own = [&] {
          while (qnext < nit && own[it_front[qnext]]) ++qnext;
        };
        size_t from = 0;
        for (int l = lvl; l < P.nlevels; ++l) {
          const size_t mid = panel_end[l - lvl], to = level_end[l - lvl];
          out.insert(out.end(), tf.begin() + from, tf.begin() + mid);
          long long room = (long long)h->spanel_fold_room - (long long)(mid - from);
          for (skip_own(); room > 0 && qnext < nit && P.sn_level[it_front[qnext]] <= l; skip_own()) {
            out.push_back(filler(qnext++));
            --room;
          }
          out.insert(out.end(), tf.begin() + mid, tf.begin() + to);
          from = to;
        }
        for (skip_own(); qnext < nit; skip_own()) out.push_back(filler(qnext++));
        tf.swap(out);
        lds = std::max(lds, sp_lds_pre);
        h->sp_folded = true;
      }
      h->ftop_level = lvl;
      h->ftop_count = (int)tf.size();
      h->ftop_lds = lds;
      for (int l = 0; l < lvl; ++l) {
        LevelInfo& lm = h->levels[l];
        if (lm.mini_cnt == 0) continue;
        const int s = P.level_sn[P.level_ptr[l]];
        auto mini = [&](int role, int part) {
          TopFItem t;
          memset(&t, 0, sizeof(t));
          t.it.Loff = sn[s].Loff;
          t.it.Uoff = sn[s].Uoff;
          t.it.w = sn[s].w;
          t.it.r = sn[s].r;
          t.it.part = part;
          t.it.nchild = sn[s].child_end - sn[s].child_begin;
          t.it.pd = pulls[s];
          t.role = role;
          t.front = s;
          t.part2 = 0;
          t.nwait = t.it.nchild;
          for (int k = 0; k < t.nwait; ++k) t.wait_id[k] = P.child_idx[sn[s].child_begin + k];
          t.crows = 64;
          t.prows = panel_rows(1);
          t.post = 1;
          t.xoff = xoff[s];
          t.target = (sn[s].r - sn[s].w + t.prows - 1) / t.prows;
          return t;
        };
        lm.mini_off = (long long)tf.size();
        tf.push_back(mini(0, 0));
        for (int b = 0; b < (sn[s].r - sn[s].w + panel_rows(1) - 1) / panel_rows(1); ++b) tf.push_back(mini(1, b));
        lm.mini_cnt = (int)(tf.size() - (size_t)lm.mini_off);
        lm.mini_lds = std::max(lm.lds_pivot, lm.lds_panel);
      }
      if ((rc = upload(h, h->d_tfitems, tf))) return rc;
    }
  }
  {
    h->fused_solve = false;
    h->n_sitems = 0;
    h->n_sliced = 0;
    bool ok = h->solve_fused && ns > 0;
    for (int s2 = 0; s2 < ns && ok; ++s2) ok = sn[s2].w >= 1 && (h->solve_slices || sn[s2].r <= 1024);
    if (ok) {
      std::vector<SolveItem> si;
      std::vector<long long> xuoff;
      std::vector<int> xinvoff;
      std::vector<int> fx0(ns, 0), fx1(ns, 0);
      std::vector<long long> fpoff(ns, 0);
      si.reserve(nit);
      long long spf = 0, spart = 0;
      int wmax = 1;
      for (int q = 0; q < nit; ++q) {
        const int s2 = it_front[q], sl = it_sl[q], nsl = it_nsl[q];
        SolveItem T;
        memset(&T, 0, sizeof(T));
        T.c0 = sn[s2].c0;
        T.w = sn[s2].w;
        T.r = sn[s2].r;
        T.uoff = sn[s2].uoff;
        T.rowoff = sn[s2].rowoff;
        T.Loff = sn[s2].Loff;
        T.plevel = sn[s2].parent >= 0 ? P.sn_level[sn[s2].parent] : -1;
        const int nch = sn[s2].child_end - sn[s2].child_begin;
        T.nchild = std::min(nch, MAXCH);
        if (sl == 0) {
          fx0[s2] = (int)xuoff.size();
          fpoff[s2] = spart;
          spart += (long long)(nsl - 1) * T.w;
        }
        for (int k = 0; k < nch; ++k) {
          const int ch = P.child_idx[sn[s2].child_begin + k];
          if (k < MAXCH) {
            T.c_uoff[k] = sn[ch].uoff;
            T.c_invoff[k] = sn[ch].pad1;
          } else if (sl == 0) {
            xuoff.push_back(sn[ch].uoff);
            xinvoff.push_back(sn[ch].pad1);
          }
        }
        if (sl == 0) fx1[s2] = (int)xuoff.size();
        T.xbegin = fx0[s2];
        T.xend = fx1[s2];
        T.sl = sl;
        T.nsl = nsl;
        T.poff = fpoff[s2];
        T.a0 = it_a0[q];
        T.a1 = it_a1[q];
        const int ro = (sl == 0 ? T.w : 0) + (T.a1 - T.a0);
        T.Qf = std::max(1, std::min(T.w, 1024 / ro));
        T.Ef = (T.w + T.Qf - 1) / T.Qf;
        T.Pb = std::max(1, std::min(ro, 1024 / T.w));
        T.Eb = (ro + T.Pb - 1) / T.Pb;
        T.spf = spf;
        T.spd = spf + (long long)T.Ef * ro * T.Qf;
        spf += ((long long)T.Ef * ro * T.Qf + (sl == 0 ? T.w : 0) + 1) & ~1LL;
        wmax = std::max(wmax, T.w);
        si.push_back(T);
      }
      h->sp_lds = solve_panel_lds(wmax);
      {
        std::vector<int> lvl_begin(P.nlevels + 1, nit);
        for (int q = nit - 1; q >= 0; --q) lvl_begin[P.sn_level[it_front[q]]] = q;
        for (int l = P.nlevels - 1; l >= 0; --l)
          if (lvl_begin[l] > lvl_begin[l + 1]) lvl_begin[l] = lvl_begin[l + 1];
        for (int l = P.nlevels - 1; l >= 0; --l)
          for (int q = lvl_begin[l]; q < lvl_begin[l + 1];) {
            const int nsl = it_nsl[q];
            for (int k = nsl - 1; k >= 0; --k) {
              const SolveItem t = si[q + k];
              si.push_back(t);
            }
            q += nsl;
          }
      }
      if (h->sp_lds <= 160 * 1024) {
        if ((rc = upload(h, h->d_sitems, si))) return rc;
        if ((rc = upload(h, h->d_sxuoff, xuoff))) return rc;
        if ((rc = upload(h, h->d_sxinvoff, xinvoff))) return rc;
        cold_tick("  upload_plan: descriptors, items, solve lists");
        HCHECK(h, h->d_SPf.ensure(std::max<size_t>((size_t)spf * sizeof(double), 16)));
        HCHECK(h, hipMemsetAsync(h->d_SPf.p, 0, std::max<size_t>((size_t)spf * sizeof(double), 16), h->stream));
        cold_tick("  upload_plan: solve-panel arena");
        HCHECK(h, h->d_xhat.ensure(std::max<size_t>((size_t)P.m * sizeof(double), 16)));
        HCHECK(h, hipMemsetAsync(h->d_xhat.p, 0xFF, std::max<size_t>((size_t)P.m * sizeof(double), 16), h->stream));
        HCHECK(h, h->d_spart.ensure(std::max<size_t>((size_t)spart * sizeof(double), 16)));
        HCHECK(h, hipMemsetAsync(h->d_spart.p, 0xFF, h->d_spart.bytes, h->stream));
        HCHECK(h, hipFuncSetAttribute(reinterpret_cast<const void*>(k_build_solve_panels),
                                      hipFuncAttributeMaxDynamicSharedMemorySize, 160 * 1024));
        h->fused_solve = true;
        h->n_sitems = nit;
        for (int q = 0; q < nit; ++q) h->n_sliced += it_sl[q] == 0 && it_nsl[q] > 1;
        h->sp_bytes = (double)spf * sizeof(double);
        h->tb_nT = h->tb_ntf = h->tb_nfb = h->tb_levels = h->tb_nchunks = 0;
        h->tb_valid = false;
        if (h->top_block_after > 0 && P.nlevels >= 4) {
          std::vector<int> lcols(P.nlevels, 0), lfronts(P.nlevels, 0);
          std::vector<char> lsingle(P.nlevels, 1);
          for (int q = 0; q < nit; ++q) {
            const int l = P.sn_level[it_front[q]];
            if (it_sl[q] == 0) {
              lcols[l] += sn[it_front[q]].w;
              lfronts[l] += 1;
            }
            if (it_nsl[q] != 1 || sn[it_front[q]].w > 128) lsingle[l] = 0;
          }
          int ltop = P.nlevels, cols = 0;
          while (ltop > 1 && lsingle[ltop - 1] && lfronts[ltop - 1] <= 32 && cols + lcols[ltop - 1] <= h->top_block_max) {
            --ltop;
            cols += lcols[ltop];
          }
          bool roots_in = true;
          for (int s2 = 0; s2 < ns; ++s2)
            if (sn[s2].parent < 0 && P.sn_level[s2] < ltop) roots_in = false;
          if (P.nlevels - ltop >= 3 && roots_in && cols >= 64) {
            const int nT = cols;
            int nfb = 0;
            while (nfb < nit && P.sn_level[it_front[nfb]] < ltop) ++nfb;
            std::vector<int> tl((size_t)P.m, -1), tpos;
            tpos.reserve((size_t)nT);
            std::vector<int> tf_of(ns, -1);
            std::vector<TopFront> tfronts;
            for (int s2 = 0; s2 < ns; ++s2)
              if (P.sn_level[s2] >= ltop) {
                tf_of[s2] = (int)tfronts.size();
                tfronts.push_back(TopFront{first_item[s2], -1, (int)tpos.size(), 0});
                for (int k = 0; k < sn[s2].w; ++k) {
                  tl[(size_t)(sn[s2].c0 + k)] = (int)tpos.size();
                  tpos.push_back(sn[s2].c0 + k);
                }
              }
            for (int s2 = 0; s2 < ns; ++s2)
              if (tf_of[s2] >= 0 && sn[s2].parent >= 0) tfronts[(size_t)tf_of[s2]].parent = tf_of[sn[s2].parent];
            std::vector<std::vector<long long>> src((size_t)nT);
            bool ok_tb = (int)tpos.size() == nT;
            for (int s2 = 0; s2 < ns && ok_tb; ++s2) {
              if (tf_of[s2] >= 0 || sn[s2].parent < 0 || tf_of[sn[s2].parent] < 0) continue;
              const int u = sn[s2].r - sn[s2].w;
              for (int a = 0; a < u; ++a) {
                const int i = tl[(size_t)P.sn_rows[(size_t)sn[s2].rowoff + sn[s2].w + a]];
                if (i < 0) {
                  ok_tb = false;
                  break;
                }
                src[(size_t)i].push_back(sn[s2].uoff + a);
              }
            }
            {
// ... 199 lines not shown
```

sleqp_amd/csrc/runtime_queue.inc:

```
struct TurnState {
  std::mutex mu;
  hipEvent_t last = nullptr;
  hipfact_handle* owner = nullptr;
  std::atomic<int> live{0};
};
static TurnState g_turn[16];
static hipfact_handle* g_trace_handles[8] = {nullptr};
struct Turn {
  hipfact_handle* h;
  bool counted = false, held = false;
  explicit Turn(hipfact_handle* h_) : h(h_) {
    if (h->capturing) return;
    counted = true;
    if (h->turn_depth++ > 0) return;
    TurnState& T = g_turn[h->device & 15];
    static const bool off = getenv("HIPFACT_NO_TURNS") != nullptr;
    if (off || T.live.load(std::memory_order_acquire) <= 1 || !h->ev_turn) return;
    T.mu.lock();
    held = true;
    if (T.last && T.owner != h) {
      (void)hipStreamWaitEvent(h->stream, T.last, 0);
      h->turn_waits++;
    }
  }
// ... 5 lines not shown
    if (hipEventRecord(h->ev_turn, h->stream) == hipSuccess) {
      T.last = h->ev_turn;
      T.owner = h;
    }
    T.mu.unlock();
  }
  Turn(const Turn&) = delete;
  Turn& operator=(const Turn&) = delete;
};
static void turn_join(hipfact_handle* h) {
  TurnState& T = g_turn[h->device & 15];
  std::lock_guard<std::mutex> g(T.mu);
  if (T.live.fetch_add(1, std::memory_order_acq_rel) == 1) (void)hipDeviceSynchronize();
  for (auto& g : g_trace_handles)
    if (!g) {
      g = h;
      break;
    }
}
static void turn_leave(hipfact_handle* h) {
  TurnState& T = g_turn[h->device & 15];
  std::lock_guard<std::mutex> g(T.mu);
  T.live.fetch_sub(1, std::memory_order_acq_rel);
  for (auto& g : g_trace_handles)
    if (g == h) g = nullptr;
  if (T.owner == h) {
    T.owner = nullptr;
    T.last = nullptr;
  }
}

static DecideIn decide_in(hipfact_handle* h, int col = -1);
static inline bool diag_inactive_needed(const hipfact_handle* h) {
  const Plan& P = h->plan;
  return P.saddle && P.m > 0 && ((h->maps_on && h->n_inactive > 0) || P.n_late > 0);
}
static inline bool row_scale_in_sequence(const hipfact_handle* h) {
  const Plan& P = h->plan;
  return P.saddle && P.n > 0 && P.m > 0;
}
static inline bool dataflow_factor(const hipfact_handle* h) { return h->debug_phases == 15 && !h->no_dataflow; }
static inline bool tree_solve(const hipfact_handle* h) { return h->fused_solve && !h->no_dataflow; }
static inline bool tree_delivers_verdict(const hipfact_handle* h) { return tree_solve(h) && h->plan.m > 0 && h->plan.saddle; }
static inline bool graph_route(const hipfact_handle* h) { return h->use_graph && !h->prof.on && h->debug_phases == 15; }
static inline const int* cmap_or_null(const hipfact_handle* h) { return (h->maps_on || h->plan.n_late > 0) ? h->d_cmap.as<int>() : nullptr; }
static inline bool masked_rows(const hipfact_handle* h) { return h->nd > 0 || h->plan.n_late > 0; }
static inline size_t arena_fill_bytes(const Plan& P) {
  return (size_t)P.L_size * sizeof(double) + (size_t)4 * P.nsuper * sizeof(int);
}
static inline int row_scale_grid(long long m, size_t fill_bytes) {
  const long long nz16 = (long long)((fill_bytes + 15) / 16);
  const int for_fill = (int)std::min<long long>(2048, std::max<long long>(1, nz16 / (FB * 8)));
  return std::max(nblocks(m * 16), for_fill);
}
static int place_rows(int m, const int* Ar_ptr, size_t fill_bytes, int classes, ClassBounds& cb) {
  return place_ranges((long long)m, FB / RL, Ar_ptr, LONG_ROW, classes, row_scale_grid(m, fill_bytes), (long long)((fill_bytes + 15) / 16), cb);
}
static void place_front_end(hipfact_handle* h) {
  const Plan& P = h->plan;
  h->rs_grid = place_rows(P.m, P.Ar_ptr.data(), arena_fill_bytes(P), h->xcd_classes, h->rs_place);
}
template <bool CH>
static void launch_schur(hipfact_handle* h, const LevelInfo& li, int pull) {
  h->prof.next_fl = li.schur_flops;
  if (li.nD <= 0) return;
  const FrontItem* fit = h->d_fitems.as<FrontItem>() + li.itD;
  if (li.pair == 2)
    LAUNCH(PC_FACTOR_D, k_front_schur_pair, dim3(li.nD), dim3(FB), li.lds_schur, fit, h->d_L.as<double>(),
           h->d_U.as<double>(), li.pd);
  else
    LAUNCH(PC_FACTOR_D, k_front_schur<CH>, dim3(li.nD), dim3(FB), li.lds_schur, fit, h->d_L.as<double>(),
           h->d_U.as<double>(), h->d_inv.as<int>(), h->d_rel.as<int>(), h->d_pullx.as<PullDesc>(), pull);
}
static int factor_enqueue(hipfact_handle* h) {
  Turn turn(h);
  const Plan& P = h->plan;
  hipStream_t st = h->stream;
  const size_t fill_bytes = arena_fill_bytes(P);
  const bool fill_rides = row_scale_in_sequence(h);
  if (!fill_rides) {
    HCHECK(h, hipMemsetAsync(h->d_info.p, 0, INFO_BYTES, st));
    if (P.L_size > 0 && fill_bytes > 0) {
      prof_begin(h, PC_MEMSET);
      HCHECK(h, hipMemsetAsync(h->d_L.p, 0, fill_bytes, st));
      prof_end(h);
    }
  }
  const long long nM = (long long)P.Mi.size();
  const int* vmap = h->maps_on ? h->d_vmap.as<int>() : nullptr;
  double* kprod = h->maps_on ? h->d_Kprod.as<double>() : h->d_Ksc.as<double>();
  if (fill_rides) {
    {
      const long long nz16 = (long long)((fill_bytes + 15) / 16);
      const bool masked = masked_rows(h);
      const double* kin = h->vals_ride ? h->vals_ride : h->d_Kval.as<double>();
      if (h->n_rseg > 0)
        LAUNCH(PC_GATHER, k_long_row_norm, dim3(std::min(h->n_rseg, 4096)), dim3(FB), 0, h->n_rseg, h->d_rseg.as<LongSeg>(),
               h->d_Ar_col.as<int>(), h->d_Ar_src.as<int>(), kin, vmap,
               masked ? h->d_dmask.as<int>() : nullptr, P.n_late > 0 ? 1 : 0, h->equilibrate ? 1 : 0,
               h->d_dscale.as<double>(), h->d_segpart.as<double>(), h->d_segcnt.as<unsigned int>());
      LAUNCH(PC_GATHER, k_row_scale, dim3(h->rs_grid), dim3(FB), 0, P.m,
             h->d_Ar_ptr.as<int>(), h->d_Ar_col.as<int>(), h->d_Ar_src.as<int>(), kin, vmap,
             masked ? h->d_dmask.as<int>() : nullptr, h->d_perm.as<int>(), P.n_late > 0 ? P.my : -1,
             h->equilibrate ? 1 : 0, h->d_dscale.as<double>(),
             h->d_Ar_val.as<double>(), masked ? h->d_Ar_full.as<double>() : nullptr, h->d_Ksc.as<double>(), kprod,
             h->vals_ride ? h->d_Kval.as<double>() : nullptr, (long long)P.nnzK,
             reinterpret_cast<double2*>(h->d_L.p), nz16, h->d_info.as<int>(), h->n_rseg,
             h->d_rseg.as<LongSeg>(), decide_in(h), h->decide_rides ? 1 : 0, h->rs_place);
    }
  }
  if (nM > 0) {
    if (P.saddle) {
#define MVALS_LAUNCH(IDX, PK)                                                                                       \
  LAUNCH(PC_MVALS, (k_mvals_prod<IDX, PK>), dim3(nblocks(nM, 1 << 16)), dim3(FB), 0, nM, h->d_prod_ptr.as<IDX>(), \
         h->d_prod_a.as<int>(), h->d_prod_b.as<int>(), h->d_Mtarget.as<IDX>(), kprod,                                  \
         h->d_L.as<double>(), h->n_lprod,                                                                              \
         h->d_lprod.as<LongProd>(), h->d_segpart.as<double>(), h->d_segcnt.as<unsigned int>())
      if (h->idx32 && h->prod_packed)
        MVALS_LAUNCH(unsigned int, true);
      else if (h->idx32)
        MVALS_LAUNCH(unsigned int, false);
      else if (h->prod_packed)
        MVALS_LAUNCH(long long, true);
      else
        MVALS_LAUNCH(long long, false);
#undef MVALS_LAUNCH
    } else {
      LAUNCH(PC_MVALS, k_mvals_src, dim3(nblocks(nM, 1 << 16)), dim3(FB), 0, nM, h->d_src.as<int>(),
                         h->d_Mtarget.as<long long>(), h->d_Kval.as<double>(), h->d_L.as<double>());
    }
  }
  if (diag_inactive_needed(h))
    LAUNCH(PC_GATHER, k_diag_inactive, dim3(nblocks(P.m)), dim3(FB), 0, P.m, h->d_perm.as<int>(), h->d_cmap.as<int>(),
           h->d_diag_target.as<long long>(), h->d_L.as<double>());
  if (P.saddle && h->reg_delta > 0.0 && P.m > 0)
    LAUNCH(PC_GATHER, k_diag_shift, dim3(nblocks(P.m)), dim3(FB), 0, P.m, h->d_perm.as<int>(), cmap_or_null(h),
           h->d_diag_target.as<long long>(), h->d_L.as<double>(), h->reg_delta);
  const bool dataflow = dataflow_factor(h);
  const int lsplit = dataflow ? std::min(h->ftop_level, P.nlevels) : P.nlevels;
  if (h->mini_x_bytes > 0 && dataflow)
    HCHECK(h, hipMemsetAsync(h->d_xarena.as<double>() + h->mini_x_off, 0xFF, h->mini_x_bytes, st));
  for (int l = 0; l < lsplit; ++l) {
    const LevelInfo& li = h->levels[l];
    const int* it = h->d_items.as<int>();
    const int pull = (li.pull && h->debug_phases == 15) ? 1 : 0;
    if (li.nA > 0 && (h->debug_phases & 1) && !pull)
      LAUNCH(PC_FACTOR_A, k_front_assemble, dim3(li.nA), dim3(1024), li.lds_asm, h->d_sn.as<SnDesc>(), it + li.itA, li.nparts,
             h->d_L.as<double>(), h->d_U.as<double>(), h->d_rel.as<int>(), h->d_child.as<int>());
    if (li.split && li.mini_cnt > 0 && dataflow && h->ftop_count > 0) {
      int* flm = reinterpret_cast<int*>(h->d_L.as<double>() + P.L_size);
      LAUNCH(PC_FACTOR_B, k_factor_top, dim3(li.mini_cnt), dim3(512), li.mini_lds,
             h->d_tfitems.as<TopFItem>() + li.mini_off, h->d_L.as<double>(), h->d_U.as<double>(), h->d_info.as<int>(),
             h->d_inv.as<int>(), h->d_rel.as<int>(), flm, flm + P.nsuper, flm + 2 * P.nsuper, h->d_xarena.as<double>(),
             nullptr, nullptr);
      launch_schur<false>(h, li, pull);
    } else if (li.split && h->debug_phases == 15) {
      const FrontItem* fit = h->d_fitems.as<FrontItem>();
#define SPLIT_LAUNCHES(CH)                                                                                              \
  LAUNCH(PC_FACTOR_B, k_front_pivot<CH>, dim3(li.count), dim3(512), li.lds_pivot, fit + li.itB, h->d_L.as<double>(),   \
         h->d_U.as<double>(), h->d_info.as<int>(), h->d_inv.as<int>(), h->d_rel.as<int>(), h->d_pullx.as<PullDesc>(), \
         pull);                                                                                                        \
  if (li.nC > 0)                                                                                                       \
    LAUNCH(PC_FACTOR_C, k_front_panel<CH>, dim3(li.nC), dim3(li.panel_threads), li.lds_panel, fit + li.itC,            \
           h->d_L.as<double>(), h->d_U.as<double>(), h->d_inv.as<int>(), h->d_rel.as<int>(),                          \
           h->d_pullx.as<PullDesc>(), pull);                                                                           \
  launch_schur<CH>(h, li, pull);
      if (li.chain) {
        SPLIT_LAUNCHES(true)
      } else {
        SPLIT_LAUNCHES(false)
      }
#undef SPLIT_LAUNCHES
    } else {
      LAUNCH(PC_FACTOR, k_factor_level, dim3(li.count), dim3(FB), li.lds_factor, h->d_sn.as<SnDesc>(),
             h->d_level_sn.as<int>() + li.begin, h->d_L.as<double>(), h->d_U.as<double>(), h->d_rel.as<int>(),
             h->d_child.as<int>(), h->d_info.as<int>(), h->debug_phases);
    }
  }
  if (lsplit < P.nlevels) {
    int* fl = reinterpret_cast<int*>(h->d_L.as<double>() + P.L_size);
    LAUNCH(PC_FACTOR_T, k_factor_top, dim3(h->ftop_count), dim3(512), h->ftop_lds, h->d_tfitems.as<TopFItem>(),
           h->d_L.as<double>(), h->d_U.as<double>(), h->d_info.as<int>(), h->d_inv.as<int>(), h->d_rel.as<int>(), fl,
           fl + P.nsuper, fl + 2 * P.nsuper, h->d_xarena.as<double>(),
           h->sp_folded ? h->d_sitems.as<SolveItem>() : nullptr, h->sp_folded ? h->d_SPf.as<double>() : nullptr);
  }
  if (tree_solve(h) && !(h->sp_folded && lsplit < P.nlevels) && h->n_sitems > 0)
    LAUNCH(PC_SPANEL, k_build_solve_panels, dim3(h->n_sitems), dim3(SPB), h->sp_lds, h->d_sitems.as<SolveItem>(),
           h->d_L.as<double>(), h->d_SPf.as<double>());
  HCHECK(h, hipGetLastError());
  return dense_setup_async(h);
}

template <class F>
static int run_cached(hipfact_handle* h, int kind, const void* b, void* z, F enqueue, int passes = 0);

static void flush_decide(hipfact_handle* h);
static void drop_graphs(hipfact_handle* h);
static int reset_dataflow_state(hipfact_handle* h);

static int factor_async(hipfact_handle* h, const double* src = nullptr) {
  const Plan& P = h->plan;
  if (h->no_dataflow && h->df_retry_at >= 0 && h->num_factor >= h->df_retry_at && !cadence(h).verdict_unread() &&
      !cadence(h).verdict_outstanding() && !h->reg_retry) {
    h->no_dataflow = false;
    h->df_retry_at = -1;
    h->dataflow_rearmed++;
    drop_graphs(h);
    h->cache.clear();
    if (const int rrc = reset_dataflow_state(h)) return rrc;
  }
  const bool graphed = graph_route(h);
  const size_t src_bytes = (size_t)P.nnzK * sizeof(double);
  if (!h->reg_retry) {
    h->reg_delta = 0.0;
    h->num_perturbed = 0;
  }
  const bool ride = src && src_bytes > 0 && row_scale_in_sequence(h);
  const bool copy_first = src && src_bytes > 0 && !ride;
  if (!graphed) {
    flush_decide(h);
    if (copy_first) HCHECK(h, hipMemcpyAsync(h->d_Kval.p, src, src_bytes, hipMemcpyDeviceToDevice, h->stream));
  }
  const bool with_decide = graphed && cadence(h).verdict_outstanding();
  const bool with_inactive = diag_inactive_needed(h);
  auto enqueue_all = [&]() -> int {
    if (graphed) {
      h->decide_rides = with_decide && row_scale_in_sequence(h);
      if (with_decide && !h->decide_rides) hipLaunchKernelGGL(k_refine_decide, dim3(1), dim3(FB), 0, h->stream, decide_in(h), 1, 1);
      if (copy_first) HCHECK(h, hipMemcpyAsync(h->d_Kval.p, src, src_bytes, hipMemcpyDeviceToDevice, h->stream));
    }
    h->vals_ride = ride ? src : nullptr;
    const int frc = factor_enqueue(h);
    h->decide_rides = false;
    h->vals_ride = nullptr;
    return frc;
  };
  h->tb_valid = false;
  if (h->factored) h->solves_prev_factor = h->solves_this_factor;
  h->solves_this_factor = 0;
  const int variant = (with_decide ? 4 : 0) + (h->reg_delta > 0.0 ? 8 : 0) + (with_inactive ? 16 : 0);
  h->note('F', variant + (graphed ? 0 : 32));
  const int rc = run_cached(h, 0, graphed ? src : nullptr, nullptr, enqueue_all, variant);
  if (rc) return rc;
  h->num_factor++;
  h->sol_prefetched = false;
  h->tb_valid = false;
  h->solves_this_factor = 0;
  h->factored = true;
  h->factor_checked = false;
  h->solved = false;
  cadence(h).factor_queued(cadence_knobs(h), graphed, ctl_peek_pinned(h));
  return HIPFACT_OK;
}

static int reset_dataflow_state(hipfact_handle* h) {
  const Plan& P = h->plan;
  hipStream_t st = h->stream;
  if (h->d_xarena.p) HCHECK(h, hipMemsetAsync(h->d_xarena.p, 0xFF, h->d_xarena.bytes, st));
  if (h->d_uvec.p) HCHECK(h, hipMemsetAsync(h->d_uvec.p, 0xFF, std::max<size_t>((size_t)P.u_size * sizeof(double), 16), st));
  if (h->d_ysol.p) HCHECK(h, hipMemsetAsync(h->d_ysol.p, 0xFF, std::max<size_t>((size_t)2 * P.m * sizeof(double), 16), st));
  if (h->d_xhat.p) HCHECK(h, hipMemsetAsync(h->d_xhat.p, 0xFF, std::max<size_t>((size_t)P.m * sizeof(double), 16), st));
  if (h->d_spart.p) HCHECK(h, hipMemsetAsync(h->d_spart.p, 0xFF, h->d_spart.bytes, st));
  if (h->d_tb_xhat.p) HCHECK(h, hipMemsetAsync(h->d_tb_xhat.p, 0xFF, h->d_tb_xhat.bytes, st));
  if (h->d_tb_gathered.p) HCHECK(h, hipMemsetAsync(h->d_tb_gathered.p, 0, 16, st));
  if (h->d_epoch.p) HCHECK(h, hipMemsetAsync(h->d_epoch.p, 0, 16, st));
  HCHECK(h, hipMemsetAsync(h->d_info.p, 0, INFO_BYTES, st));
  HCHECK(h, hipMemsetAsync(h->d_ctl.p, 0, sizeof(RefineCtl), st));
  HCHECK(h, hipStreamSynchronize(st));
  memset(h->h_ctl.p, 0, sizeof(RefineCtl));
  cadence(h).slots_reset();
  return HIPFACT_OK;
}

static void trace_timeout(hipfact_handle* h, const char* msg) {
  static const bool on = getenv("HIPFACT_TRACE_TIMEOUT") != nullptr;
  if (!on) return;
  const Plan& P = h->plan;
  std::vector<int> fl((size_t)4 * P.nsuper);
  if (h->d_L.p && hipMemcpy(fl.data(), h->d_L.as<double>() + P.L_size, fl.size() * sizeof(int), hipMemcpyDeviceToHost) == hipSuccess)
    for (int l = 0; l < P.nlevels; ++l) {
      int open = 0, nb = 0, nc = 0, nd = 0;
      for (int q = P.level_ptr[l]; q < P.level_ptr[l + 1]; ++q) {
        const int sn = P.level_sn[q];
        open += fl[sn] == 0;
        nb += fl[sn];
        nc += fl[P.nsuper + sn];
        nd += fl[2 * P.nsuper + sn];
      }
      fprintf(stderr, "   level %2d fronts %4d  without pivot flag %4d  sums bdone %d cdone %d ddone %d\n", l,
              P.level_ptr[l + 1] - P.level_ptr[l], open, nb, nc, nd);
    }
  fprintf(stderr, "[hipfact %p] %s; factorisation %ld, solve %ld, turn waits %lld, handles on the device %d\n", (void*)h, msg,
          (long)h->num_factor, (long)h->live_cad.solve_seq, h->turn_waits, g_turn[h->device & 15].live.load());
  fprintf(stderr, "   first solve workgroup that timed out: %d (items %d, top block %d: %d below)\n",
          h->info_host[INFO_TIMEOUT_WG] ? (1 << 30) - h->info_host[INFO_TIMEOUT_WG] : -1, h->n_sitems, (int)h->tb_valid, h->tb_nfb);
  for (hipfact_handle* o : g_trace_handles)
    if (o && o != h) {
      fprintf(stderr, "   other handle %p: factorisations %ld, analyses %ld, turn waits %lld, launches %u, last:", (void*)o,
              (long)o->num_factor, (long)o->analyses, o->turn_waits, o->n_notes);
      for (unsigned k = o->n_notes > 6 ? o->n_notes - 6 : 0; k < o->n_notes; ++k) fprintf(stderr, " %c%d", o->notes[k & 63].kind, o->notes[k & 63].key);
      fprintf(stderr, "\n");
    }
  fprintf(stderr, "   last launches:");
  for (unsigned k = h->n_notes > 64 ? h->n_notes - 64 : 0; k < h->n_notes; ++k)
    fprintf(stderr, " %c%d", h->notes[k & 63].kind, h->notes[k & 63].key);
  fprintf(stderr, "\n");
}

enum class Phase { factor, solve };
static int check_info(hipfact_handle* h, Phase phase = Phase::factor, bool* switched = nullptr) {
  if (switched) *switched = false;
  HCHECK(h, hipMemcpyAsync(h->h_info.p, h->d_info.p, INFO_BYTES, hipMemcpyDeviceToHost, h->stream));
  HCHECK(h, hipStreamSynchronize(h->stream));
  memcpy(h->info_host, h->h_info.p, INFO_WORDS * sizeof(int));
  if (phase == Phase::factor) {
    unsigned long long mm[2];
    memcpy(mm, h->h_info.as<char>() + INFO_WORDS * sizeof(int), sizeof(mm));
    const unsigned long long nlo = ~mm[0];
    double lo, hi;
    memcpy(&lo, &nlo, 8);
    memcpy(&hi, &mm[1], 8);
    h->pivot_ratio = (mm[1] == 0ull) ? 1.0 : ((lo > 0.0 && hi >= lo) ? hi / lo : INFINITY);
  }
  const bool factor_was_checked = h->factor_checked;
  h->factor_checked = true;
  if (h->fake_timeouts > 0) {
    --h->fake_timeouts;
    h->info_host[INFO_TIMEOUT] += 1;
  }
  char buf[200];
  if (h->info_host[INFO_TIMEOUT] != 0) {
    snprintf(buf, sizeof buf, "dependency wait timed out inside the single-launch %s kernels (%d waits)",
             phase == Phase::solve ? "solve" : "factorisation", h->info_host[INFO_TIMEOUT]);
    const bool in_solve = phase == Phase::solve && factor_was_checked;
    if (!in_solve) h->factored = false;
    h->solved = false;
    const int rc = reset_dataflow_state(h);
// ... 670 lines not shown
```

sleqp_amd/csrc/runtime_types.inc:

```
namespace hipfact {

struct DevBuf {
  void* p = nullptr;
  size_t bytes = 0;
  DevBuf() = default;
  DevBuf(const DevBuf&) = delete;
  DevBuf& operator=(const DevBuf&) = delete;
  DevBuf(DevBuf&& o) noexcept : p(o.p), bytes(o.bytes) {
    o.p = nullptr;
    o.bytes = 0;
  }
  DevBuf& operator=(DevBuf&& o) noexcept {
    if (this != &o) {
      release();
      p = o.p;
      bytes = o.bytes;
      o.p = nullptr;
      o.bytes = 0;
    }
    return *this;
  }
  ~DevBuf() { release(); }
  void release() {
    if (p) (void)hipFree(p);
    p = nullptr;
    bytes = 0;
  }
  hipError_t ensure(size_t n) {
    if (n <= bytes) return hipSuccess;
    release();
    if (n == 0) return hipSuccess;
    hipError_t e = hipMalloc(&p, n);
    if (e == hipSuccess) bytes = n;
    return e;
  }
  template <class T>
  T* as() const {
    return static_cast<T*>(p);
  }
};

struct PinBuf {
  void* p = nullptr;
  size_t bytes = 0;
  ~PinBuf() {
    if (p) (void)hipHostFree(p);
  }
  hipError_t ensure(size_t n) {
    if (n <= bytes) return hipSuccess;
    if (p) (void)hipHostFree(p);
    p = nullptr;
    bytes = 0;
    hipError_t e = hipHostMalloc(&p, n, hipHostMallocDefault);
    if (e == hipSuccess) bytes = n;
    return e;
  }
  template <class T>
  T* as() const {
    return static_cast<T*>(p);
  }
};

struct LevelInfo {
  int begin = 0, count = 0;
  size_t lds_factor = 0, lds_fwd = 0, lds_bwd = 0;
  bool split = false;
  bool pull = false;
  bool chain = false;
  int nparts = 1;
  long long itA = 0;
  long long itB = 0, itC = 0, itD = 0;
  int nA = 0, nC = 0, nD = 0;
  int panel_threads = 512;
  size_t lds_pivot = 0, lds_panel = 0, lds_schur = 0, lds_asm = 0, lds_solve_max = 0;
  int pair = 0;
  PairDesc pd;
  double schur_flops_full = 0.0, pair_flops_done = 0.0;
  bool compactD = false;
  double schur_flops = 0.0;
  long long mini_off = 0;
  int mini_cnt = 0;
  size_t mini_lds = 0;
};

enum ProfClass { PC_MEMSET = 0, PC_MVALS, PC_GATHER, PC_FACTOR, PC_FACTOR_A, PC_FACTOR_B, PC_FACTOR_C, PC_FACTOR_D, PC_FACTOR_T, PC_FWD, PC_BWD, PC_RHS, PC_XUPD, PC_RESID, PC_AXPY, PC_PERM, PC_SPANEL, PC_TREE, PC_COUNT };
static const char* const kProfNames[PC_COUNT] = {"memset", "mvals", "gather", "factor", "factorA", "factorB", "factorC",
                                                 "factorD", "factorT", "fwd", "bwd", "rhs", "xupd", "resid", "axpy", "perm",
                                                 "spanel", "tree"};

struct Prof {
  bool on = false;
  std::vector<hipEvent_t> ev;
  std::vector<int> cls;
  size_t used = 0;
  double ms[PC_COUNT] = {0};
  double max_ms[PC_COUNT] = {0};
  std::vector<double> fl;
  double next_fl = 0.0;
  std::vector<std::pair<double, double>> tagged;
  long cnt[PC_COUNT] = {0};
  ~Prof() {
    for (hipEvent_t e : ev) (void)hipEventDestroy(e);
  }
};

}

using namespace hipfact;

static thread_local std::string g_create_error;

constexpr size_t CG_DOTS_DOUBLES =
    (size_t)(5 * CG_BLOCKS + 3 * (DOT_BLOCKS > 1024 ? DOT_BLOCKS : 1024)) > (size_t)(2 * 3 * DOT_BLOCKS + 8 + 1024)
        ? (size_t)(5 * CG_BLOCKS + 3 * (DOT_BLOCKS > 1024 ? DOT_BLOCKS : 1024))
        : (size_t)(2 * 3 * DOT_BLOCKS + 8 + 1024);

struct GraphEntry {
  int kind;
  const void* b;
  void* z;
  int passes;
  hipGraphExec_t exec;
};

struct GraphList {
  std::vector<GraphEntry> v;
  GraphList() = default;
  GraphList(const GraphList&) = delete;
  GraphList& operator=(const GraphList&) = delete;
  GraphList(GraphList&& o) noexcept : v(std::move(o.v)) { o.v.clear(); }
  GraphList& operator=(GraphList&& o) noexcept {
    if (this != &o) {
      clear();
      v = std::move(o.v);
      o.v.clear();
    }
    return *this;
  }
  ~GraphList() { clear(); }
  void clear() {
    for (auto& g : v) (void)hipGraphExecDestroy(g.exec);
    v.clear();
  }
  size_t size() const { return v.size(); }
  std::vector<GraphEntry>::iterator begin() { return v.begin(); }
  std::vector<GraphEntry>::iterator end() { return v.end(); }
  void push_back(const GraphEntry& g) { v.push_back(g); }
};

struct FactorMemo {
  bool solved = false;
  long solves_this_factor = 0;
};

struct PlanState : FactorMemo {
  Plan plan;
  bool have_plan = false, factored = false;
  bool factor_checked = false;
  bool prod_packed = false;
  bool idx32 = false;
  unsigned long long key_hash = 0;
  bool from_jacobian = false;
  std::vector<int> Jp, Ji;
  std::vector<int> sidx;
  int m_struct = 0;
  bool maps_on = false;
  int N_ext = 0;
  int n_inactive = 0;
  int n_bounds = 0;
  unsigned long long use_stamp = 0;
  hipfact::FactorCadence factor_cad;
  hipfact::PlanCadence plan_cad;
  GraphList graphs;
  int ftop_level = 1 << 30, ftop_count = 0;
  size_t ftop_lds = 0;
  long long mini_x_off = 0;
  size_t mini_x_bytes = 0;
  double ent_fused = 0, ent_split = 0, rows_fused = 0, rows_split = 0;
  std::vector<LevelInfo> levels;
  DevBuf d_sn, d_level_sn, d_rows, d_rel, d_child, d_Mtarget, d_prod_ptr, d_prod_a, d_prod_b, d_src;
  DevBuf d_items, d_fitems, d_inv, d_tfitems, d_pullx;
  DevBuf d_perm, d_Ar_ptr, d_Ar_col, d_Ar_src, d_Ar_val, d_Kp, d_Ki, d_Kc_y, d_Tp, d_Ti, d_Tsrc;
  DevBuf d_xarena;
  DevBuf d_ysol;
  DevBuf d_Kval, d_L, d_U, d_uvec, d_y, d_rhs, d_sol, d_res;
  DevBuf d_Ksc, d_Kprod, d_dscale, d_vmap, d_cmap, d_diag_target, d_sidx, d_srow, d_jtarget;
  bool fused_solve = false;
  size_t sp_lds = 0;
  double sp_bytes = 0;
  DevBuf d_SPf, d_sitems, d_xhat, d_sxuoff, d_sxinvoff, d_epoch, d_spart;
  int n_sitems = 0;
  int n_sliced = 0;
  int n_resorted = 0;
  int last_rhs_in_tree = 0, last_xupd_in_tree = 0, last_xupd_blocks = 0;
  int tb_nT = 0, tb_ntf = 0, tb_nfb = 0, tb_levels = 0, tb_nchunks = 0;
  bool tb_valid = false;
  long solves_prev_factor = 1 << 20;
  DevBuf d_tb_gathered;
  DevBuf d_tb_zd, d_tb_items, d_tb_xtf, d_tb_tpos, d_tb_tl, d_tb_gptr, d_tb_gsrc, d_tb_xhat, d_tb_xd, d_tb_fronts,
      d_tb_chunks, d_tb_dsrc, d_tb_dinv, d_tb_zp;
  int nd = 0, dense_cap = 0;
  DevBuf d_dmask, d_dcols, d_Bq, d_Zq, d_dtmp, d_dG, d_dMinv, d_dw, d_dfix;
  DevBuf d_Ar_full;
  DevBuf d_rseg, d_cseg, d_lprod, d_segpart, d_segcnt;
  int n_rseg = 0, n_cseg = 0, n_lprod = 0;
  ClassBounds rs_place = {};
  int rs_grid = 1;
  int dealt_multi = 0;
  int n_lrows = 0;
  DevBuf d_mY, d_mU, d_mR, d_mB;
  DevBuf d_mitems, d_mslab, d_mcnt;
  std::vector<int> mitem_ptr;
  int mitems_for = -1;
  int n_mcut = 0, n_mslices = 0;
  size_t mcnt_bytes = 0;
  DevBuf d_xvec;
  DevBuf d_xmvec;
  DevBuf d_cblk, d_cwords, d_cused;

  PlanState() = default;
  PlanState(PlanState&&) = default;
  PlanState& operator=(PlanState&&) = default;
};

#define VTABLE_SUPERSET_TYPES
#include "vtable_superset.inc"
#undef VTABLE_SUPERSET_TYPES

struct SingleSolveMemo {
  const double* last_b = nullptr;
  double* last_z = nullptr;
  RefineCtl last_ctl = {1, 0, 0, 0, 0, 0, 0.0, 0.0, 0.0, 0.0};
  bool sol_prefetched = false;
  long num_solve = 0;
};

struct hipfact_handle : PlanState, SingleSolveMemo {
  std::atomic<int> refcount{1};
  int device = 0;
  hipStream_t stream = nullptr;
  hipStream_t side = nullptr;
  hipEvent_t ev_fork = nullptr, ev_join = nullptr;
  hipEvent_t ev_turn = nullptr;
  int turn_depth = 0;
  struct LaunchNote { char kind; int key; };
  LaunchNote notes[64];
  unsigned n_notes = 0;
  void note(char kind, int key) { notes[n_notes++ & 63] = LaunchNote{kind, key}; }
  long long turn_waits = 0;
  bool capturing = false;
  std::string error;
  PlanParams prm;
  std::vector<std::unique_ptr<PlanState>> cache;
  int plan_cache_max = 4;
  bool chain_fuse = true;
  bool solve_slices = true;
  bool speculate = true;
  bool xupd_fused = true;
  bool rhs_fused = true;
  bool spanel_fold = true;
  int spanel_fold_room = 224;
  bool sp_folded = false;
  bool solve_fused = true;
  bool assemble_superset = true;
  bool spmv_stream = true;
  long long spmv_stream_min = 4 << 20;
  bool exact_pattern = false;
  bool superset_vtable = true;
  std::unique_ptr<VirtualJ> vj{new VirtualJ};
  DevBuf d_kin, d_vsrc;
  DevBuf d_retry_b;
  long vtable_retries = 0;
  long dense_fallbacks = 0;
  bool jdev_valid = false;
  unsigned long long jdev_hash = 0;
  int jdev_n = 0, jdev_nnz = 0;
  unsigned long long use_clock = 0;
  long plan_swaps = 0;
  int refine_steps = 1;
  int refine_max = 10;
  bool refine_adaptive = true;
  double refine_tol = 1e-10;
  double fail_omega = 1e-8;
  bool static_pivot = true;
  double static_delta = 1e-8;
  double reg_delta = 0.0;
  bool reg_retry = false;
  int num_perturbed = 0;
  long static_pivot_runs = 0;
  std::string warning;
  bool equilibrate = true;
  bool decide_lazy = true;
  hipfact::SolveCadence solve_cad;
  hipfact::LiveCadence live_cad;
  int refine_check_every = 8;
  int refine_check_backoff = 2;
  int refine_check_max = 64;
  double pivot_ratio = 1.0;
  bool no_solve_retry = false;
  long dense_probes = 0;
  bool decide_rides = false;
  const double* vals_ride = nullptr;
  bool use_graph = true;
  bool no_dataflow = false;
  int fake_timeouts = 0;
  long dataflow_fallbacks = 0;
  int df_retry_every = 256;
  long df_retry_at = -1;
  long dataflow_rearmed = 0;
  int debug_phases = 15;
  int solve_whole_max = 48;
  bool factor_hint_peek = true;
  int top_block_breakeven = 48;
  bool chain_pairs = true;
  int n_pairs = 0;
  long long pair_extra = 0;
  double schur_flops_max = 0.0;
  bool check_launches = false, launch_reported = false;
  double* x_dot_out = nullptr;
  int x_dot_blocks = 0;
  int xupd_blocks = 256;
  bool solve_sorted = true;
  int xcd_classes = 8;
  int factor_top_max = 160;
  int factor_top_levels = 1 << 20;
  int factor_top_max_u = 1024;
  int factor_top_fine = 12;
  int top_block_after = 2;
  int top_block_max = 2048;
  long tb_builds = 0;
  bool factor_top_head = true;
  int factor_top_fused = 30;
  int factor_top_fused32 = 12;
  int factor_top_fused_u = 256;
// ... 138 lines not shown
```

Before: 1499 factor+solve/s.

## Precompute per-item child index maps for top factor kernel and prefetch Schur gathers

At plan time, builds a per-work-item slot table holding the first two children's inverse-index entries (pivot columns, panel rows, Schur tile rows and columns) and uploads it to the device. k_factor_top then reads these directly instead of chasing pc.inv per child, and panel items write their index tables before waiting on children. The Schur tile path issues gathers for the first two children before the flag wait and adds them afterward, overlapping the load latency with the dependency wait. This costs extra registers and a 2KB map per item, and it ties correctness to the host-built maps staying in sync with the item layout.

```diff
diff --git a/include/hipfact.h b/include/hipfact.h
--- a/include/hipfact.h
+++ b/include/hipfact.h
@@ -207,6 +207,8 @@
 int hipfact_debug_place_items(int nfronts, const int* counts, int classes, int* order, int* lost);
 
 int hipfact_debug_multi_slices(int u, int slice_rows, int* tile_bounds , int cap);
+
+int hipfact_debug_top_maps(int nitems, const int* desc, const int* inv, long long ninv, int* slots);
 
 int hipfact_debug_extra_rule(int nblocks, int npasses, const double* dn, const double* zn, int pass_cap, int* applied,
                              int* status, double* ferr, double* rho);
diff --git a/sleqp_amd/_lib.py b/sleqp_amd/_lib.py
--- a/sleqp_amd/_lib.py
+++ b/sleqp_amd/_lib.py
@@ -27,7 +27,7 @@
     "hipfact_assemble_kkt", "hipfact_reduced_matrix", "hipfact_spmat_create", "hipfact_spmat_update_values", "hipfact_spmat_free",
     "hipfact_spmat_mult_vec", "hipfact_spmat_mult_vec_trans", "hipfact_spmat_mult_vec_sym",
     "hipfact_spmat_mult_device", "hipfact_steihaug_solve", "hipfact_tr_solve", "hipfact_tr_solve_ex", "hipfact_lsqr_solve", "hipfact_tridiag_tr", "hipfact_set_option", "hipfact_get_info", "hipfact_debug_copy", "hipfact_debug_pool_selftest",
-    "hipfact_debug_place_rows", "hipfact_debug_place_items", "hipfact_debug_multi_slices", "hipfact_debug_refine_cadence", "hipfact_plan_create",
+    "hipfact_debug_place_rows", "hipfact_debug_place_items", "hipfact_debug_multi_slices", "hipfact_debug_top_maps", "hipfact_debug_refine_cadence", "hipfact_plan_create",
     "hipfact_plan_free", "hipfact_plan_error", "hipfact_plan_array", "hipfact_plan_scalar",
 ]
 
@@ -111,6 +111,8 @@
         lib.hipfact_debug_place_items.argtypes = [ci, vp, ci, vp, vp]
     if hasattr(lib, "hipfact_debug_multi_slices"):
         lib.hipfact_debug_multi_slices.argtypes = [ci, ci, vp, ci]
+    if hasattr(lib, "hipfact_debug_top_maps"):
+        lib.hipfact_debug_top_maps.argtypes = [ci, vp, vp, C.c_longlong, vp]
     if hasattr(lib, "hipfact_debug_refine_cadence"):
         lib.hipfact_debug_refine_cadence.argtypes = [vp, ci, vp, vp]
     lib.hipfact_plan_create.argtypes = [ci, vp, vp, vp, C.POINTER(vp)]
diff --git a/sleqp_amd/csrc/abi_options.inc b/sleqp_amd/csrc/abi_options.inc
--- a/sleqp_amd/csrc/abi_options.inc
+++ b/sleqp_amd/csrc/abi_options.inc
@@ -314,6 +314,30 @@
   return ns;
 }
 
+int hipfact_debug_top_maps(int nitems, const int* desc, const int* inv, long long ninv, int* slots) {
+  if (nitems < 0 || ninv < 0 || (nitems > 0 && (!desc || !slots)) || (ninv > 0 && !inv)) return HIPFACT_EINVAL;
+  for (int q = 0; q < nitems; ++q) {
+    const int* d = desc + 12 * (size_t)q;
+    if (d[1] < 0 || d[2] < d[1] || d[6] < 0 || d[8] < 0 || d[8] > MAXCH || (d[0] == 1 && d[3] < 0)) return HIPFACT_EINVAL;
+    for (int c = 0; c < std::min(d[8], TOPMAP_CH); ++c)
+      if (d[9 + c] < 0 || (long long)d[9 + c] + d[2] > ninv) return HIPFACT_EINVAL;
+    TopFItem T;
+    memset(&T, 0, sizeof(T));
+    T.role = d[0];
+    T.it.w = d[1];
+    T.it.r = d[2];
+    T.it.part = d[3];
+    T.part2 = d[4];
+    T.crows = d[5];
+    T.prows = d[6];
+    T.post = d[7];
+    T.it.pd.n = d[8];
+    for (int c = 0; c < TOPMAP_CH; ++c) T.it.pd.invoff[c] = d[9 + c];
+    fill_top_map_slot(T, inv, slots + (size_t)q * TOPMAP_STRIDE);
+  }
+  return HIPFACT_OK;
+}
+
 int hipfact_debug_refine_cadence(const int* knobs, int nevents, const double* events, long long* rows) {
   using namespace hipfact;
   if (!knobs || nevents < 0 || (nevents > 0 && (!events || !rows))) return HIPFACT_EINVAL;
@@ -471,7 +495,7 @@
   INFO("num_passes", h->solve_cad.num_passes) INFO("last_omega", h->last_ctl.omega) INFO("last_iters", h->last_ctl.iters)
   INFO("last_status", h->last_ctl.status) INFO("last_tol", h->last_ctl.tol) INFO("kappa_est", h->last_ctl.kappa)
   INFO("refine_inline", h->factor_cad.refine_inline) INFO("refine_tol", h->refine_tol) INFO("equilibrate", h->equilibrate)
-  INFO("factor_top_level", h->ftop_level) INFO("factor_top_count", h->ftop_count) INFO("solve_timeouts", h->h_info.p ? h->h_info.as<int>()[INFO_TIMEOUT] : 0)
+  INFO("factor_top_level", h->ftop_level) INFO("factor_top_count", h->ftop_count) INFO("factor_top_map_bytes", h->ftop_map_bytes) INFO("solve_timeouts", h->h_info.p ? h->h_info.as<int>()[INFO_TIMEOUT] : 0)
   INFO("top_level", 1 << 30)
   INFO("use_graph", h->use_graph) INFO("num_graphs", h->graphs.size()) INFO("max_r", P.max_r) INFO("max_w", P.max_w) INFO("refine_steps", h->refine_steps)
   INFO("schur_flops_max_level", h->schur_flops_max)
diff --git a/sleqp_amd/csrc/device_types.h b/sleqp_amd/csrc/device_types.h
--- a/sleqp_amd/csrc/device_types.h
+++ b/sleqp_amd/csrc/device_types.h
@@ -61,6 +61,9 @@
   int head;
   int wait_head[MAXCH];
 };
+constexpr int TOPMAP_CH = 2;
+constexpr int TOPMAP_STRIDE = 512;
+constexpr int TOPMAP_ROWS = 256;
 
 struct SolveItem {
   long long spf, spd;
diff --git a/sleqp_amd/csrc/hipfact.hip b/sleqp_amd/csrc/hipfact.hip
--- a/sleqp_amd/csrc/hipfact.hip
+++ b/sleqp_amd/csrc/hipfact.hip
@@ -28,6 +28,7 @@
 #include "kernels_decl.h"
 #include "xcd_place.h"
 #include "multi_slices.h"
+#include "top_maps.h"
 #include "refine_cadence.h"
 #include "condest_rule.h"
 #include "dd_arith.h"
diff --git a/sleqp_amd/csrc/kernels_factor_top.inc b/sleqp_amd/csrc/kernels_factor_top.inc
--- a/sleqp_amd/csrc/kernels_factor_top.inc
+++ b/sleqp_amd/csrc/kernels_factor_top.inc
@@ -33,10 +33,15 @@
                                                    const int* __restrict__ inv, const int* __restrict__ rel,
                                                    int* __restrict__ bdone, int* __restrict__ cdone,
                                                    int* __restrict__ ddone, double* __restrict__ xarena,
-                                                   const SolveItem* __restrict__ sitems, double* __restrict__ SPf) {
+                                                   const SolveItem* __restrict__ sitems, double* __restrict__ SPf,
+                                                   const int* __restrict__ maps) {
   extern __shared__ __attribute__((aligned(16))) double lds[];
   const TopFItem& T = items[blockIdx.x];
   const FrontItem& S = T.it;
+  const int* __restrict__ slot = maps + (size_t)blockIdx.x * TOPMAP_STRIDE;
+  const int m0 = slot[threadIdx.x];
+  const int mrow = TOPMAP_ROWS + 16 * (threadIdx.x >> 6) + (threadIdx.x & 15);
+  const int mr[TOPMAP_CH] = {slot[mrow], slot[mrow + 128]};
   TRW(0);
 #ifdef HIPFACT_TRACE
   if (threadIdx.x == 0 && blockIdx.x < TRACE_WGS) g_trace[blockIdx.x * 8 + 7] = T.role * 100000 + T.front;
@@ -88,7 +93,7 @@
       }
   }
   if (T.role == 0) {
-    dev_pivot_block<false, false, true>(c, info, 15, pc, cw);
+    dev_pivot_block<false, false, true>(c, info, 15, pc, cw, no_more(), m0, true);
     dev_store_pivot_block(c);
     TRW(2);
     flag_publish_add(&bdone[T.front]);
@@ -105,12 +110,14 @@
     }
   } else if (T.role == 1) {
     TRW(5);
-    cw.wait();
     int* invl = reinterpret_cast<int*>(c.A + c.wp * c.lda);
+    if (threadIdx.x < 128 * TOPMAP_CH && (int)(threadIdx.x >> 7) < pc.n && (int)(threadIdx.x & 127) < c.wp)
+      invl[(threadIdx.x >> 7) * c.wp + (threadIdx.x & 127)] = m0;
 #pragma unroll
-    for (int ch = 0; ch < MAXCH; ++ch)
+    for (int ch = TOPMAP_CH; ch < MAXCH; ++ch)
       if (ch < pc.n)
         for (int k = threadIdx.x; k < c.wp; k += blockDim.x) invl[ch * c.wp + k] = (k < c.w) ? pc.inv[ch][k] : -1;
+    cw.wait();
     const int wv = threadIdx.x >> 6;
     const int cstep = T.prows == 64 ? 2 : 1;
     const int R0 = c.w + T.prows * S.part + 16 * (cstep == 2 ? (wv >> 1) : wv);
@@ -121,6 +128,8 @@
       const int R1 = c.w + T.prows * S.part + 16 * wv;
       const int Rs = mine ? R1 : c.r;
       dev_panel_rows_load<true>(c, Rs, pc, pv, cis);
+#pragma unroll
+      for (int ch = 0; ch < TOPMAP_CH; ++ch) cis[ch] = mr[ch];
       __syncthreads();
       dev_panel_rows_gather<true>(c, pc, invl, pv, cis);
       TRW(1);
@@ -131,6 +140,8 @@
       return;
     }
     dev_panel_rows_load(c, R0, pc, pv, cis);
+#pragma unroll
+    for (int ch = 0; ch < TOPMAP_CH; ++ch) cis[ch] = mr[ch];
     __syncthreads();
     dev_panel_rows_gather(c, pc, invl, pv, cis);
     if (c.Xa) {
@@ -167,7 +178,7 @@
       const int ij = team ? T.part2 : S.part;
       double* SI = c.A + (size_t)team * (2 * 64 * KC + 64 * MAXCH);
       dev_schur_tile<false>(c, SI, SI + 64 * KC, ij < 0 ? -1 : (ij >> 16), ij & 0xffff, S.nchild == 0, pc,
-                            threadIdx.x & 255, &cdone[T.front], T.target, info);
+                            threadIdx.x & 255, &cdone[T.front], T.target, info, no_more(), m0, true);
     }
     if (c.Xa)
       for (int e = T.sidx * 512 + threadIdx.x; e < c.wp * c.wp; e += T.scount * 512) sent_f64(c.Xa + e);
diff --git a/sleqp_amd/csrc/kernels_front_pivot.inc b/sleqp_amd/csrc/kernels_front_pivot.inc
--- a/sleqp_amd/csrc/kernels_front_pivot.inc
+++ b/sleqp_amd/csrc/kernels_front_pivot.inc
@@ -389,7 +389,8 @@
 
 template <bool ROWINV, bool CHAIN = false, bool V2 = false>
 __device__ __forceinline__ void dev_pivot_block(const FrontCtx& c, int* __restrict__ info, int phases, const PullCtx& pc,
-                                                const ChildWait& cw, const PullMore pm = no_more()) {
+                                                const ChildWait& cw, const PullMore pm = no_more(), const int slot0 = -1,
+                                                const bool has_slot = false) {
   const int tid = threadIdx.x, lane = tid & 63, wave = tid >> 6;
   const int nw = blockDim.x >> 6;
   const int li = lane & 15, lk = lane >> 4;
@@ -405,7 +406,8 @@
     int* invb = reinterpret_cast<int*>(Yp + 16 * lda + 32);
     int iv[MAXCH];
 #pragma unroll
-    for (int ch = 0; ch < MAXCH; ++ch) iv[ch] = (ch < pc.n && tid < w) ? pc.inv[ch][tid] : -1;
+    for (int ch = 0; ch < MAXCH; ++ch)
+      iv[ch] = (ch < pc.n && tid < w && !(has_slot && ch < TOPMAP_CH)) ? pc.inv[ch][tid] : -1;
     const int i1 = tid & 127, kq1 = tid >> 7;
     double v1[4];
 #pragma unroll
@@ -426,7 +428,9 @@
       }
 #pragma unroll
     for (int ch = 0; ch < MAXCH; ++ch)
-      if (ch < pc.n && tid < wp) invb[ch * wp + tid] = iv[ch];
+      if (ch < pc.n && tid < wp && !(has_slot && ch < TOPMAP_CH)) invb[ch * wp + tid] = iv[ch];
+    if (has_slot && tid < 128 * TOPMAP_CH && (tid >> 7) < pc.n && (tid & 127) < wp)
+      invb[(tid >> 7) * wp + (tid & 127)] = slot0;
     __syncthreads();
     if constexpr (!CHAIN) {
       int o1[MAXCH][4], o2[2][2][8];
diff --git a/sleqp_amd/csrc/kernels_front_update.inc b/sleqp_amd/csrc/kernels_front_update.inc
--- a/sleqp_amd/csrc/kernels_front_update.inc
+++ b/sleqp_amd/csrc/kernels_front_update.inc
@@ -14,10 +14,10 @@
 constexpr int KC = 32;
 constexpr int SCB = 64;
 __device__ __forceinline__ void schur_tile_gather(const PullCtx& pc, const int* invs, int i0, int j0, int li, int lk,
-                                                  double (&uv)[2][2][4]) {
+                                                  double (&uv)[2][2][4], const int first = 0) {
 #pragma unroll
   for (int ch = 0; ch < MAXCH; ++ch)
-    if (ch < pc.n) {
+    if (ch >= first && ch < pc.n) {
       const double* __restrict__ Uc = pc.Uc[ch];
       const int uc = pc.uc[ch];
       const int* iv = invs + 128 * ch;
@@ -47,12 +47,47 @@
           for (int q = 0; q < 4; ++q) uv[x][y][q] += g[x][y][q];
     }
 }
+__device__ __forceinline__ unsigned schur_tile_gather_request(const PullCtx& pc, const int ch, const int* invs, int i0,
+                                                              int j0, int li, int lk, double (&g)[2][2][4]) {
+  const double* __restrict__ Uc = pc.Uc[ch];
+  const int uc = pc.uc[ch];
+  const int* iv = invs + 128 * ch;
+  int ci[2], cj[2][4];
+#pragma unroll
+  for (int y = 0; y < 2; ++y) ci[y] = iv[i0 + 16 * y + li];
+#pragma unroll
+  for (int x = 0; x < 2; ++x)
+#pragma unroll
+    for (int q = 0; q < 4; ++q) cj[x][q] = iv[64 + j0 + 16 * x + lk + 4 * q];
+  unsigned okm = 0;
+#pragma unroll
+  for (int x = 0; x < 2; ++x)
+#pragma unroll
+    for (int y = 0; y < 2; ++y)
+#pragma unroll
+      for (int q = 0; q < 4; ++q) {
+        const bool ok = ci[y] >= 0 && cj[x][q] >= 0 && ci[y] >= cj[x][q];
+        g[x][y][q] = Uc[ok ? ci[y] + (long long)cj[x][q] * uc : 0];
+        okm |= ok ? 1u << (8 * x + 4 * y + q) : 0u;
+      }
+  return okm;
+}
+__device__ __forceinline__ void schur_tile_gather_add(const double (&g)[2][2][4], const unsigned okm,
+                                                      double (&uv)[2][2][4]) {
+#pragma unroll
+  for (int x = 0; x < 2; ++x)
+#pragma unroll
+    for (int y = 0; y < 2; ++y)
+#pragma unroll
+      for (int q = 0; q < 4; ++q) uv[x][y][q] += ((okm >> (8 * x + 4 * y + q)) & 1u) ? g[x][y][q] : 0.0;
+}
 
 template <bool DD_IN_LDS, bool CHAIN = false>
 __device__ __forceinline__ void dev_schur_tile(const FrontCtx& c, double* SI, double* SJ, int I, int J, bool assign,
                                                const PullCtx& pc, const int tid, int* wait_addr = nullptr,
                                                int wait_target = 0, int* info = nullptr,
-                                               const PullMore pm = no_more()) {
+                                               const PullMore pm = no_more(), const int slot0 = -1,
+                                               const bool has_slot = false) {
   const int lane = tid & 63, wave = tid >> 6;
   const int li = lane & 15, lk = lane >> 4;
   const int w = c.w, r = c.r, u = c.u;
@@ -85,18 +120,28 @@
     for (int h = 0; h < 2; ++h) {
       const int ch = (tid >> 7) + 2 * h, idx = tid & 127;
       const int gi = (idx < 64) ? 64 * I + idx : 64 * J + idx - 64;
-#pragma unroll
-      for (int cc = 0; cc < MAXCH; ++cc)
-        if (cc == ch && cc < pc.n && gi < u && !ghost) ivr[h] = pc.inv[cc][w + gi];
-    }
-  }
+      if (has_slot && h == 0) {
+        ivr[0] = slot0;
+      } else {
+#pragma unroll
+        for (int cc = 0; cc < MAXCH; ++cc)
+          if (cc == ch && cc < pc.n && gi < u && !ghost) ivr[h] = pc.inv[cc][w + gi];
+      }
+    }
+  }
+  double gd[2][2][2][4];
+  unsigned gok[2] = {0u, 0u};
   if (wait_addr) {
     if (pc.n > 0) {
       invs[tid] = ivr[0];
       invs[tid + 256] = ivr[1];
     }
     __syncthreads();
-    if (!idle) schur_tile_gather(pc, invs, i0, j0, li, lk, uv);
+    if (!idle) {
+#pragma unroll
+      for (int cc = 0; cc < 2; ++cc)
+        if (cc < pc.n) gok[cc] = schur_tile_gather_request(pc, cc, invs, i0, j0, li, lk, gd[cc]);
+    }
     TRW(5);
     flag_wait_ge(wait_addr, wait_target, info);
     TRW(1);
@@ -154,7 +199,14 @@
       }
     }
   }
-  if (!wait_addr) {
+  if (wait_addr) {
+    if (!idle) {
+#pragma unroll
+      for (int cc = 0; cc < 2; ++cc)
+        if (cc < pc.n) schur_tile_gather_add(gd[cc], gok[cc], uv);
+      if (pc.n > 2) schur_tile_gather(pc, invs, i0, j0, li, lk, uv, 2);
+    }
+  } else {
     if (!idle) schur_tile_gather(pc, invs, i0, j0, li, lk, uv);
     for (int nx = CHAIN ? pc.next : -1; nx >= 0;) {
       const PullCtx px = make_pull(pm.more[nx], pm.U, pm.inv, pm.rel, 1);
diff --git a/sleqp_amd/csrc/runtime_plan.inc b/sleqp_amd/csrc/runtime_plan.inc
--- a/sleqp_amd/csrc/runtime_plan.inc
+++ b/sleqp_amd/csrc/runtime_plan.inc
@@ -464,6 +464,7 @@
   {
     h->ftop_level = 1 << 30;
     h->ftop_count = 0;
+    h->ftop_map_bytes = 0;
     int lvl = P.nlevels;
     while (lvl > 0) {
       const LevelInfo& li = h->levels[lvl - 1];
@@ -741,6 +742,10 @@
         lm.mini_lds = std::max(lm.lds_pivot, lm.lds_panel);
       }
       if ((rc = upload(h, h->d_tfitems, tf))) return rc;
+      std::vector<int> tfmaps(tf.size() * (size_t)TOPMAP_STRIDE);
+      fill_top_maps(tf.data(), tf.size(), inv.data(), tfmaps.data());
+      h->ftop_map_bytes = tfmaps.size() * sizeof(int);
+      if ((rc = upload(h, h->d_tfmaps, tfmaps))) return rc;
     }
   }
   {
diff --git a/sleqp_amd/csrc/runtime_queue.inc b/sleqp_amd/csrc/runtime_queue.inc
--- a/sleqp_amd/csrc/runtime_queue.inc
+++ b/sleqp_amd/csrc/runtime_queue.inc
@@ -181,7 +181,7 @@
       LAUNCH(PC_FACTOR_B, k_factor_top, dim3(li.mini_cnt), dim3(512), li.mini_lds,
              h->d_tfitems.as<TopFItem>() + li.mini_off, h->d_L.as<double>(), h->d_U.as<double>(), h->d_info.as<int>(),
              h->d_inv.as<int>(), h->d_rel.as<int>(), flm, flm + P.nsuper, flm + 2 * P.nsuper, h->d_xarena.as<double>(),
-             nullptr, nullptr);
+             nullptr, nullptr, h->d_tfmaps.as<int>() + li.mini_off * TOPMAP_STRIDE);
       launch_schur<false>(h, li, pull);
     } else if (li.split && h->debug_phases == 15) {
       const FrontItem* fit = h->d_fitems.as<FrontItem>();
@@ -211,7 +211,8 @@
     LAUNCH(PC_FACTOR_T, k_factor_top, dim3(h->ftop_count), dim3(512), h->ftop_lds, h->d_tfitems.as<TopFItem>(),
            h->d_L.as<double>(), h->d_U.as<double>(), h->d_info.as<int>(), h->d_inv.as<int>(), h->d_rel.as<int>(), fl,
            fl + P.nsuper, fl + 2 * P.nsuper, h->d_xarena.as<double>(),
-           h->sp_folded ? h->d_sitems.as<SolveItem>() : nullptr, h->sp_folded ? h->d_SPf.as<double>() : nullptr);
+           h->sp_folded ? h->d_sitems.as<SolveItem>() : nullptr, h->sp_folded ? h->d_SPf.as<double>() : nullptr,
+           h->d_tfmaps.as<int>());
   }
   if (tree_solve(h) && !(h->sp_folded && lsplit < P.nlevels) && h->n_sitems > 0)
     LAUNCH(PC_SPANEL, k_build_solve_panels, dim3(h->n_sitems), dim3(SPB), h->sp_lds, h->d_sitems.as<SolveItem>(),
diff --git a/sleqp_amd/csrc/runtime_types.inc b/sleqp_amd/csrc/runtime_types.inc
--- a/sleqp_amd/csrc/runtime_types.inc
+++ b/sleqp_amd/csrc/runtime_types.inc
@@ -174,12 +174,13 @@
   GraphList graphs;
   int ftop_level = 1 << 30, ftop_count = 0;
   size_t ftop_lds = 0;
+  size_t ftop_map_bytes = 0;
   long long mini_x_off = 0;
   size_t mini_x_bytes = 0;
   double ent_fused = 0, ent_split = 0, rows_fused = 0, rows_split = 0;
   std::vector<LevelInfo> levels;
   DevBuf d_sn, d_level_sn, d_rows, d_rel, d_child, d_Mtarget, d_prod_ptr, d_prod_a, d_prod_b, d_src;
-  DevBuf d_items, d_fitems, d_inv, d_tfitems, d_pullx;
+  DevBuf d_items, d_fitems, d_inv, d_tfitems, d_tfmaps, d_pullx;
   DevBuf d_perm, d_Ar_ptr, d_Ar_col, d_Ar_src, d_Ar_val, d_Kp, d_Ki, d_Kc_y, d_Tp, d_Ti, d_Tsrc;
   DevBuf d_xarena;
   DevBuf d_ysol;
diff --git a/sleqp_amd/csrc/top_maps.h b/sleqp_amd/csrc/top_maps.h
--- /dev/null
+++ b/sleqp_amd/csrc/top_maps.h
@@ -0,0 +1,45 @@
+#pragma once
+#include <cstddef>
+
+#include "device_types.h"
+
+namespace hipfact {
+
+inline void fill_top_map_slot(const TopFItem& T, const int* inv, int* slot) {
+  for (int e = 0; e < TOPMAP_STRIDE; ++e) slot[e] = -1;
+  const int w = T.it.w, r = T.it.r, u = r - w;
+  const int n = T.it.pd.n < TOPMAP_CH ? T.it.pd.n : TOPMAP_CH;
+  if (T.role == 0 || T.role == 1) {
+    for (int c = 0; c < n; ++c)
+      for (int k = 0; k < 128 && k < w; ++k) slot[128 * c + k] = inv[T.it.pd.invoff[c] + k];
+  }
+  if (T.role == 1) {
+    for (int c = 0; c < n; ++c)
+      for (int v = 0; v < 8; ++v) {
+        const int strip = (!T.post && T.prows == 64) ? (v >> 1) : v;
+        if (T.post && 16 * v >= T.prows) continue;
+        for (int l = 0; l < 16; ++l) {
+          const long long R = (long long)w + (long long)T.prows * T.it.part + 16 * strip + l;
+          if (R < r) slot[TOPMAP_ROWS + 128 * c + 16 * v + l] = inv[T.it.pd.invoff[c] + R];
+        }
+      }
+  }
+  if (T.role == 2 && T.crows == 128) {
+    for (int team = 0; team < 2; ++team) {
+      const int ij = team ? T.part2 : T.it.part;
+      if (ij < 0) continue;
+      const int I = ij >> 16, J = ij & 0xffff;
+      for (int c = 0; c < n; ++c)
+        for (int i = 0; i < 128; ++i) {
+          const long long g = i < 64 ? 64LL * I + i : 64LL * J + i - 64;
+          if (g < u) slot[256 * team + 128 * c + i] = inv[T.it.pd.invoff[c] + w + g];
+        }
+    }
+  }
+}
+
+inline void fill_top_maps(const TopFItem* items, size_t count, const int* inv, int* out) {
+  for (size_t q = 0; q < count; ++q) fill_top_map_slot(items[q], inv, out + q * (size_t)TOPMAP_STRIDE);
+}
+
+}
```

Measured after the change: 1502 factor+solve/s, median of 2. Within noise of the previous version (+0.2%).
